# zhenfeizhang/falcon-r1cs

Measured on AMD Instinct MI355X. Metric: falcon1024_verify_with_ntt_r1cs_witnesses_per_sec, higher is better.
Workload: dtype u32

## Files before the change

falcon-r1cs_amd/csrc/frw_fq29.h:

```cpp
#pragma once
#include <hip/hip_runtime.h>
#include <stdint.h>

namespace frw {

constexpr int NLQ = 14;
constexpr uint32_t MQ29 = (1u << 29) - 1u;

struct Fq29 { uint32_t l[NLQ]; };
struct LimbsQ { uint32_t l[NLQ]; };

constexpr uint32_t Q32_[12] = {0xffffaaabu, 0xb9feffffu, 0xb153ffffu, 0x1eabfffeu, 0xf6b0f624u, 0x6730d2a0u,
                               0xf38512bfu, 0x64774b84u, 0x434bacd7u, 0x4b1ba7b6u, 0x397fe69au, 0x1a0111eau};
constexpr LimbsQ make_kq29(uint32_t K)
{
    uint32_t w[14] = {0, 0, 0, 0, 0, 0, 0, 0, 0, 0, 0, 0, 0, 0};
    uint64_t carry = 0;
    for (int k = 0; k < 12; k++) {
        const uint64_t t = (uint64_t)K * Q32_[k] + carry;
        w[k] = (uint32_t)t;
        carry = t >> 32;
    }
    w[12] = (uint32_t)carry;
    LimbsQ r{};
// ... 382 lines not shown
{
    uint32_t y[12], x[12];
    fq_pack(fq_reduce(a), y);
    if (fq_inv_words31(y, x)) return fq_mul(fq_unpack(x), fq_const(FQ29_R3));
    return fq_inv_binary(a);
}
__host__ __device__ inline Fq29 fq_inv_binary(const Fq29 &a)
{
    uint32_t u[12], v[12], x1[12], x2[12];
    fq_pack(fq_reduce(a), u);
#pragma unroll
    for (int k = 0; k < 12; k++) { v[k] = Q32_[k]; x1[k] = k == 0 ? 1u : 0u; x2[k] = 0u; }
#pragma nounroll
    for (int round = 0; round < 2 * 382; round++) {
        uint32_t any = 0;
#pragma unroll
        for (int k = 0; k < 12; k++) any |= u[k];
#if defined(__HIP_DEVICE_COMPILE__)
        if (__builtin_amdgcn_ballot_w64(any != 0) == 0) break;
#else
        if (any == 0) break;
#endif
        const uint32_t odd = 0u - (u[0] & 1u);
        uint32_t d[12], e[12], f[12];
        uint32_t borrow = 0;
#pragma unroll
        for (int k = 0; k < 12; k++) d[k] = sub_b(u[k], v[k], borrow);
        const uint32_t less = 0u - borrow, take = odd & less;
        borrow = 0;
#pragma unroll
        for (int k = 0; k < 12; k++) e[k] = sub_b(x1[k], x2[k], borrow);
        const uint32_t below = 0u - borrow;
        uint32_t carry = 0;
#pragma unroll
        for (int k = 0; k < 12; k++) e[k] = add_c(e[k], Q32_[k] & below, carry);
        borrow = 0;
#pragma unroll
        for (int k = 0; k < 12; k++) f[k] = sub_b(Q32_[k], e[k], borrow);
        borrow = 0;
#pragma unroll
        for (int k = 0; k < 12; k++) {
            const uint32_t neg = sub_b(d[k] ^ less, less, borrow);
            const uint32_t tu = u[k], tx = x1[k];
            u[k] = (odd & neg) | (~odd & tu);
            v[k] = (take & tu) | (~take & v[k]);
            x1[k] = (odd & ((less & f[k]) | (~less & e[k]))) | (~odd & tx);
            x2[k] = (take & tx) | (~take & x2[k]);
        }
        const uint32_t xodd = 0u - (x1[0] & 1u);
        carry = 0;
#pragma unroll
        for (int k = 0; k < 12; k++) x1[k] = add_c(x1[k], Q32_[k] & xodd, carry);
#pragma unroll
        for (int k = 0; k < 12; k++) {
            u[k] = (u[k] >> 1) | (k + 1 < 12 ? u[k + 1] << 31 : 0u);
            x1[k] = (x1[k] >> 1) | (k + 1 < 12 ? x1[k + 1] << 31 : 0u);
        }
    }
    return fq_mul(fq_unpack(x2), fq_const(FQ29_R3));
}

struct Fq2_29 { Fq29 c0, c1; };
__host__ __device__ __forceinline__ Fq2_29 fq2_mul(const Fq2_29 &a, const Fq2_29 &b)
{
    const Fq29 m0 = fq_mul(a.c0, b.c0), m1 = fq_mul(a.c1, b.c1), m2 = fq_mul(fq_add(a.c0, a.c1), fq_add(b.c0, b.c1));
    Fq2_29 r;
    r.c0 = fq_sub<4>(m0, m1);
    r.c1 = fq_sub<4>(fq_sub<4>(m2, m0), m1);
    return r;
}
__host__ __device__ __forceinline__ Fq2_29 fq2_sqr(const Fq2_29 &a)
{
    Fq2_29 r;
    r.c0 = fq_mul(fq_add(a.c0, a.c1), fq_sub<1024>(a.c0, a.c1));
    const Fq29 t = fq_mul(a.c0, a.c1);
    r.c1 = fq_add(t, t);
    return r;
}

struct FqField {
    typedef Fq29 El;
    static constexpr uint32_t K_MUL = 4, K_2MUL = 4, K_X = 16, K_Y = 16;
    static constexpr uint32_t K_AFFINE = K_MUL;
    static constexpr int WORDS = NLQ, ARK_WORDS = 12, LANES = 1;
    __host__ __device__ static __forceinline__ El mul(const El &a, const El &b) { return fq_mul(a, b); }
    __host__ __device__ static __forceinline__ El sqr(const El &a) { return fq_sqr(a); }
    template <uint32_t KC> __host__ __device__ static __forceinline__ El mul_sub(const El &a, const El &b, const El &c, const El &d) { return fq_mul_sub<KC>(a, b, c, d); }
    __host__ __device__ static __forceinline__ El add(const El &a, const El &b) { return fq_add(a, b); }
    template <uint32_t K> __host__ __device__ static __forceinline__ El sub(const El &a, const El &b) { return fq_sub<K>(a, b); }
    template <uint32_t K> __host__ __device__ static __forceinline__ El neg(const El &a) { return fq_neg<K>(a); }
    __host__ __device__ static __forceinline__ El zero() { return fq_zero(); }
    __host__ __device__ static __forceinline__ El one() { return fq_const(FQ29_ONE); }
    __host__ __device__ static __forceinline__ bool is_zero(const El &a) { return fq_is_zero(a); }
    __host__ __device__ static inline El inv(const El &a) { return fq_inv(a); }
    __host__ __device__ static __forceinline__ El from_ark(const uint32_t *w) { return fq_from_ark(w); }
    __host__ __device__ static __forceinline__ void to_ark(const El &a, uint32_t *w) { fq_to_ark(a, w); }
    __host__ __device__ static __forceinline__ void store(const El &a, uint32_t *w)
    {
#pragma unroll
        for (int k = 0; k < NLQ; k++) w[k] = a.l[k];
    }
    __host__ __device__ static __forceinline__ El load(const uint32_t *w)
    {
        El a;
#pragma unroll
        for (int k = 0; k < NLQ; k++) a.l[k] = w[k];
        return a;
    }
};
struct Fq2Field {
    typedef Fq2_29 El;
    static constexpr uint32_t K_MUL = 16, K_2MUL = 64, K_X = 256, K_Y = 64;
    static constexpr uint32_t K_AFFINE = K_MUL;
    static constexpr int WORDS = 2 * NLQ, ARK_WORDS = 24, LANES = 1;
    __host__ __device__ static __forceinline__ El mul(const El &a, const El &b) { return fq2_mul(a, b); }
    __host__ __device__ static __forceinline__ El sqr(const El &a) { return fq2_sqr(a); }
    template <uint32_t KC> __host__ __device__ static __forceinline__ El mul_sub(const El &a, const El &b, const El &c, const El &d)
    {
        return sub<K_MUL>(fq2_mul(a, b), fq2_mul(c, d));
    }
    __host__ __device__ static __forceinline__ El add(const El &a, const El &b) { El r; r.c0 = fq_add(a.c0, b.c0); r.c1 = fq_add(a.c1, b.c1); return r; }
    template <uint32_t K> __host__ __device__ static __forceinline__ El sub(const El &a, const El &b)
    {
        El r; r.c0 = fq_sub<K>(a.c0, b.c0); r.c1 = fq_sub<K>(a.c1, b.c1); return r;
    }
    template <uint32_t K> __host__ __device__ static __forceinline__ El neg(const El &a) { El r; r.c0 = fq_neg<K>(a.c0); r.c1 = fq_neg<K>(a.c1); return r; }
    __host__ __device__ static __forceinline__ El zero() { El r; r.c0 = r.c1 = fq_zero(); return r; }
    __host__ __device__ static __forceinline__ El one() { El r; r.c0 = fq_const(FQ29_ONE); r.c1 = fq_zero(); return r; }
    __host__ __device__ static __forceinline__ bool is_zero(const El &a) { return fq_is_zero(a.c0) && fq_is_zero(a.c1); }
    __host__ __device__ static inline El inv(const El &a)
    {
        const Fq29 n = fq_inv(fq_add(fq_mul(a.c0, a.c0), fq_mul(a.c1, a.c1)));
        El r; r.c0 = fq_mul(a.c0, n); r.c1 = fq_mul(fq_neg<1024>(a.c1), n); return r;
    }
    __host__ __device__ static __forceinline__ El from_ark(const uint32_t *w) { El r; r.c0 = fq_from_ark(w); r.c1 = fq_from_ark(w + 12); return r; }
    __host__ __device__ static __forceinline__ void to_ark(const El &a, uint32_t *w) { fq_to_ark(a.c0, w); fq_to_ark(a.c1, w + 12); }
    __host__ __device__ static __forceinline__ void store(const El &a, uint32_t *w) { FqField::store(a.c0, w); FqField::store(a.c1, w + NLQ); }
    __host__ __device__ static __forceinline__ El load(const uint32_t *w) { El r; r.c0 = FqField::load(w); r.c1 = FqField::load(w + NLQ); return r; }
};

#if defined(__HIPCC__)
struct Fq2Half { Fq29 v; };
__device__ __forceinline__ uint32_t pair_swap_u32(uint32_t x)
{
    return (uint32_t)__builtin_amdgcn_mov_dpp((int)x, 0xB1 , 0xf, 0xf, true);
}
__device__ __forceinline__ Fq29 pair_swap(const Fq29 &a)
{
    Fq29 r;
#pragma unroll
    for (int i = 0; i < NLQ; i++) r.l[i] = pair_swap_u32(a.l[i]);
    return r;
}
__device__ __forceinline__ Fq29 fq_select(bool take_a, const Fq29 &a, const Fq29 &b)
{
    Fq29 r;
#pragma unroll
    for (int i = 0; i < NLQ; i++) r.l[i] = take_a ? a.l[i] : b.l[i];
    return r;
}
struct Fq2PairField {
    typedef Fq2Half El;
    static constexpr uint32_t K_MUL = 4, K_2MUL = 16, K_X = 256, K_Y = 64;
    static constexpr uint32_t K_AFFINE = 16;
    static constexpr int WORDS = 2 * NLQ, ARK_WORDS = 24, LANES = 2;
    __device__ static __forceinline__ bool odd() { return (threadIdx.x & 1u) != 0; }
    __device__ static __forceinline__ El mul(const El &a, const El &b)
    {
        const Fq29 ap = pair_swap(a.v), bp = pair_swap(b.v);
        const bool o = odd();
        const Fq29 x = fq_select(o, ap, a.v), y = fq_select(o, a.v, fq_neg<1024>(ap));
        uint64_t col[2 * NLQ];
        fq_mul2_cols(x, b.v, y, bp, col);
        El r;
        r.v = fq_reduce_cols(col);
        return r;
    }
    __device__ static __forceinline__ El sqr(const El &a)
    {
        const Fq29 ap = pair_swap(a.v);
        const bool o = odd();
        const Fq29 x = fq_add(a.v, fq_select(o, a.v, ap)), y = fq_select(o, ap, fq_sub<1024>(a.v, ap));
        El r;
        r.v = fq_mul(x, y);
        return r;
    }
    template <uint32_t KC> __device__ static __forceinline__ El mul_sub(const El &a, const El &b, const El &c, const El &d)
    {
        return sub<K_MUL>(mul(a, b), mul(c, d));
    }
    __device__ static __forceinline__ El add(const El &a, const El &b) { El r; r.v = fq_add(a.v, b.v); return r; }
    template <uint32_t K> __device__ static __forceinline__ El sub(const El &a, const El &b) { El r; r.v = fq_sub<K>(a.v, b.v); return r; }
    template <uint32_t K> __device__ static __forceinline__ El neg(const El &a) { El r; r.v = fq_neg<K>(a.v); return r; }
    __device__ static __forceinline__ El zero() { El r; r.v = fq_zero(); return r; }
    __device__ static __forceinline__ El one() { El r; r.v = fq_select(odd(), fq_zero(), fq_const(FQ29_ONE)); return r; }
    __device__ static __forceinline__ bool is_zero(const El &a)
    {
        const uint32_t mine = fq_is_zero(a.v) ? 1u : 0u;
        return (mine & pair_swap_u32(mine)) != 0;
    }
    __device__ static inline El inv(const El &a)
    {
        const Fq29 sq = fq_sqr(a.v);
        const Fq29 n = fq_inv(fq_add(sq, pair_swap(sq)));
        El r;
        r.v = fq_mul(fq_select(odd(), fq_neg<1024>(a.v), a.v), n);
        return r;
    }
    __device__ static __forceinline__ El from_ark(const uint32_t *w) { El r; r.v = fq_from_ark(w + (odd() ? 12 : 0)); return r; }
    __device__ static __forceinline__ void to_ark(const El &a, uint32_t *w) { fq_to_ark(a.v, w + (odd() ? 12 : 0)); }
    __device__ static __forceinline__ void store(const El &a, uint32_t *w) { FqField::store(a.v, w + (odd() ? NLQ : 0)); }
    __device__ static __forceinline__ El load(const uint32_t *w) { El r; r.v = FqField::load(w + (odd() ? NLQ : 0)); return r; }
};
#endif

constexpr LimbsQ G1_GEN_X29 = {{0x0af58fd1u, 0x1662a68eu, 0x07d2c530u, 0x08993c24u, 0x1e4f4756u, 0x0c5f7ae2u, 0x0f589991u,
                                0x00dc570eu, 0x121b54f5u, 0x05242b28u, 0x17442464u, 0x0ee8a0cdu, 0x1f591099u, 0x00000009u}};
constexpr LimbsQ G1_GEN_Y29 = {{0x1cd65f60u, 0x1919ce91u, 0x0da44145u, 0x0810b2ccu, 0x08f38c44u, 0x00629241u, 0x0f521d8cu,
                                0x0529cbadu, 0x0506077fu, 0x191b2712u, 0x0c587ccbu, 0x1017da2fu, 0x1c72eafau, 0x0000000bu}};
constexpr LimbsQ G2_GEN_X0_29 = {{0x085d7b9eu, 0x0d352838u, 0x124c5276u, 0x1748cfe0u, 0x10081802u, 0x0bfc6540u, 0x01ac1784u,
                                   0x11aab37fu, 0x08f338c1u, 0x19443e06u, 0x1cc29975u, 0x0a0da681u, 0x0a53e408u, 0x00000004u}};
constexpr LimbsQ G2_GEN_X1_29 = {{0x0ba695cbu, 0x1034485fu, 0x124f6eb5u, 0x0778336bu, 0x1e170b2du, 0x12164b09u, 0x1d34eb65u,
                                   0x10a72ef2u, 0x07b96a4eu, 0x194de314u, 0x0fd4fa4au, 0x0178f021u, 0x10455591u, 0x0000000bu}};
constexpr LimbsQ G2_GEN_Y0_29 = {{0x1ec793b8u, 0x1780929bu, 0x0cdd65c4u, 0x126ca64fu, 0x0f9f2f6bu, 0x09485ce0u, 0x0621fd94u,
                                   0x1e0e7efdu, 0x09ba1f86u, 0x06d0a458u, 0x1f790335u, 0x0af83757u, 0x00c11d05u, 0x0000000cu}};
constexpr LimbsQ G2_GEN_Y1_29 = {{0x014e8093u, 0x07f6c9aau, 0x19bd3883u, 0x156ca3e1u, 0x0e34898fu, 0x0840b6feu, 0x0594f57du,
                                   0x149969ecu, 0x12886b3eu, 0x1cbcbe34u, 0x1cae2f62u, 0x08f5e851u, 0x187a6c6cu, 0x00000003u}};

constexpr LimbsQ G1_ENDO_BETA29 = {{0x1195dfebu, 0x1b04e484u, 0x06026044u, 0x086070a2u, 0x1fd68858u, 0x137e9670u, 0x06871e67u,
                                    0x1e736664u, 0x083b24f6u, 0x08a70373u, 0x02a012fdu, 0x0112f94bu, 0x18a2733cu, 0x00000003u}};

template <class F> struct AffineT { typename F::El x, y; bool inf; };
template <class F> struct XyzzT { typename F::El x, y, zz, zzz; bool inf; };

template <class F> __host__ __device__ __forceinline__ XyzzT<F> pt_identity()
{
    XyzzT<F> r;
    r.x = r.y = r.zz = r.zzz = F::zero();
    r.inf = true;
    return r;
}
template <class F> __host__ __device__ __forceinline__ XyzzT<F> pt_from_affine(const AffineT<F> &p)
{
    XyzzT<F> r;
    r.x = p.x; r.y = p.y; r.zz = r.zzz = F::one();
    r.inf = p.inf;
    return r;
}
template <class F> __host__ __device__ inline XyzzT<F> pt_double(const XyzzT<F> &p)
{
    if (p.inf) return p;
    const auto u = F::add(p.y, p.y);
    const auto v = F::sqr(u), w = F::mul(u, v);
    const auto s = F::mul(p.x, v);
    const auto xx = F::sqr(p.x);
    const auto m = F::add(F::add(xx, xx), xx);
    XyzzT<F> r;
    r.x = F::template sub<F::K_2MUL>(F::sqr(m), F::add(s, s));
    r.y = F::template mul_sub<F::K_MUL>(m, F::template sub<F::K_X>(s, r.x), w, p.y);
    r.zz = F::mul(v, p.zz);
    r.zzz = F::mul(w, p.zzz);
    r.inf = false;
    return r;
}
template <class F> __host__ __device__ __forceinline__ XyzzT<F> pt_add_affine(const XyzzT<F> &p, const AffineT<F> &q)
{
    if (q.inf) return p;
    if (p.inf) return pt_from_affine(q);
    const auto u2 = F::mul(q.x, p.zz), s2 = F::mul(q.y, p.zzz);
    const auto pp_ = F::template sub<F::K_X>(u2, p.x);
    const auto rr = F::template sub<F::K_Y>(s2, p.y);
    if (F::is_zero(pp_)) {
        if (F::is_zero(rr)) return pt_double(pt_from_affine(q));
        return pt_identity<F>();
    }
    const auto pp = F::sqr(pp_), ppp = F::mul(pp_, pp), qq = F::mul(p.x, pp);
    XyzzT<F> r;
    r.x = F::template sub<F::K_2MUL>(F::template sub<F::K_MUL>(F::sqr(rr), ppp), F::add(qq, qq));
    r.y = F::template mul_sub<F::K_Y>(rr, F::template sub<F::K_X>(qq, r.x), p.y, ppp);
    r.zz = F::mul(p.zz, pp);
    r.zzz = F::mul(p.zzz, ppp);
    r.inf = false;
    return r;
}
template <class F> __host__ __device__ inline XyzzT<F> pt_add(const XyzzT<F> &p, const XyzzT<F> &q)
{
    if (q.inf) return p;
    if (p.inf) return q;
    const auto u1 = F::mul(p.x, q.zz), u2 = F::mul(q.x, p.zz), s1 = F::mul(p.y, q.zzz), s2 = F::mul(q.y, p.zzz);
    const auto pp_ = F::template sub<F::K_MUL>(u2, u1), rr = F::template sub<F::K_MUL>(s2, s1);
    if (F::is_zero(pp_)) {
        if (F::is_zero(rr)) return pt_double(p);
        return pt_identity<F>();
    }
    const auto pp = F::sqr(pp_), ppp = F::mul(pp_, pp), qq = F::mul(u1, pp);
    XyzzT<F> r;
    r.x = F::template sub<F::K_2MUL>(F::template sub<F::K_MUL>(F::sqr(rr), ppp), F::add(qq, qq));
    r.y = F::template mul_sub<F::K_MUL>(rr, F::template sub<F::K_X>(qq, r.x), s1, ppp);
    r.zz = F::mul(F::mul(p.zz, q.zz), pp);
    r.zzz = F::mul(F::mul(p.zzz, q.zzz), ppp);
    r.inf = false;
    return r;
}
template <class F> __host__ __device__ inline AffineT<F> pt_to_affine(const XyzzT<F> &p)
{
    AffineT<F> r;
    r.inf = p.inf;
    if (p.inf) { r.x = r.y = F::zero(); return r; }
    const auto inv = F::inv(F::mul(p.zz, p.zzz));
    r.x = F::mul(p.x, F::mul(inv, p.zzz));
    r.y = F::mul(p.y, F::mul(inv, p.zz));
    return r;
}

typedef AffineT<FqField> G1Affine29;
typedef XyzzT<FqField> G1Xyzz;
typedef AffineT<Fq2Field> G2Affine29;
typedef XyzzT<Fq2Field> G2Xyzz;
__host__ __device__ __forceinline__ G1Xyzz g1_identity() { return pt_identity<FqField>(); }
__host__ __device__ __forceinline__ G1Xyzz g1_from_affine(const G1Affine29 &p) { return pt_from_affine(p); }
__host__ __device__ inline G1Xyzz g1_double(const G1Xyzz &p) { return pt_double(p); }
__host__ __device__ inline G1Xyzz g1_add_affine(const G1Xyzz &p, const G1Affine29 &q) { return pt_add_affine(p, q); }
__host__ __device__ inline G1Xyzz g1_add(const G1Xyzz &p, const G1Xyzz &q) { return pt_add(p, q); }
__host__ __device__ inline G1Affine29 g1_to_affine(const G1Xyzz &p) { return pt_to_affine(p); }

}
```

falcon-r1cs_amd/csrc/frw_msm.hip:

```cpp
#include <hip/hip_runtime.h>
#include <stdint.h>
#include <algorithm>
#include <cstdlib>
#include <cstring>
#include <functional>
#include <new>
#include <mutex>
#include <vector>
#include "../../include/frw.h"
#include "frw_device.h"
#include "frw_fq29.h"
#include "frw_quad.h"
#include "frw_fr29.h"

namespace frw {

constexpr int MSM_C = 16;
constexpr int MSM_W = 16;
constexpr int MSM_BUCKETS = 1 << (MSM_C - 1);
constexpr int MSM_FOLD1_THREADS = 4096;
constexpr int MSM_FOLD_THREADS = 512;
template <class F> struct Grp {
    static constexpr int PT_WORDS = 2 * F::WORDS, BK_WORDS = 4 * F::WORDS + 4, ARK_WORDS = 2 * F::ARK_WORDS;
    static constexpr uint32_t K_AFFINE_Y = F::K_AFFINE;
// ... 358 lines not shown
#pragma unroll
        for (int k = 0; k < WIDE_TILE / 1024; k++) {
            const uint32_t i = tile0 + t + 1024u * k;
            dv[k] = i < hi ? digits[j * n + i] : 0;
            if (dv[k]) atomicAdd(&tcount[((uint32_t)(dv[k] < 0 ? -dv[k] : dv[k]) - 1u) >> 10], 1u);
        }
        __syncthreads();
        {
            uint32_t incl = t < WIDE_BINS ? tcount[t] : 0u;
            const uint32_t own = incl, lane = t & 63;
#pragma unroll
            for (int off = 1; off < 64; off <<= 1) {
                const uint32_t v = __shfl_up(incl, off, 64);
                if (lane >= (uint32_t)off) incl += v;
            }
            if (t < WIDE_BINS && lane == 63) wtotal[t >> 6] = incl;
            __syncthreads();
            if (t < WIDE_BINS) {
                uint32_t before = 0;
                for (uint32_t w_ = 0; w_ < (t >> 6); w_++) before += wtotal[w_];
                tstart[t] = before + incl - own;
            }
            __syncthreads();
        }
#pragma unroll
        for (int k = 0; k < WIDE_TILE / 1024; k++) {
            if (!dv[k]) continue;
            const uint32_t i = tile0 + t + 1024u * k, m = (uint32_t)(dv[k] < 0 ? -dv[k] : dv[k]) - 1u, bin = m >> 10;
            const uint32_t pos = tstart[bin] + atomicAdd(&tfill[bin], 1u);
            stage[pos] = make_uint2(i | (dv[k] < 0 ? 0x80000000u : 0u), m & (WIDE_BIN_BUCKETS - 1));
            sbin[pos] = (uint16_t)bin;
        }
        __syncthreads();
        const uint32_t total = tstart[WIDE_BINS - 1] + tcount[WIDE_BINS - 1];
        for (uint32_t p = t; p < total; p += 1024) {
            const uint32_t bin = sbin[p];
            coarse[gpos[bin] + (p - tstart[bin])] = stage[p];
        }
        __syncthreads();
        if (t < WIDE_BINS) gpos[t] += tcount[t];
        __syncthreads();
    }
}
constexpr int WIDE_PARTS = 32;
static_assert(WIDE_ALL_BINS % 8 == 0, "bins go to the XCDs eight at a time");
struct WidePart { size_t g; uint32_t part, lo, hi; };
__device__ __forceinline__ WidePart wide_part_of(uint32_t w, const uint32_t *__restrict__ bin_count)
{
    WidePart p;
    const uint32_t q = w >> 3;
    p.part = q % WIDE_PARTS;
    p.g = (size_t)(q / WIDE_PARTS) * 8 + (w & 7);
    const uint32_t cnt = bin_count[p.g];
    p.lo = (uint32_t)((uint64_t)cnt * p.part / WIDE_PARTS);
    p.hi = (uint32_t)((uint64_t)cnt * (p.part + 1) / WIDE_PARTS);
    return p;
}
__global__ __launch_bounds__(1024) void msm_wide_bucket_hist_kernel(const uint2 *__restrict__ coarse, const uint32_t *__restrict__ bin_count,
                                                                    const unsigned long long *__restrict__ bin_start, uint32_t *__restrict__ part_hist)
{
    __shared__ uint32_t hist[WIDE_BIN_BUCKETS];
    const WidePart p = wide_part_of(blockIdx.x, bin_count);
    const uint2 *src = coarse + bin_start[p.g];
    hist[threadIdx.x] = 0;
    __syncthreads();
    for (uint32_t i = p.lo + threadIdx.x; i < p.hi; i += 1024) atomicAdd(&hist[src[i].y], 1u);
    __syncthreads();
    part_hist[(p.g * WIDE_PARTS + p.part) * WIDE_BIN_BUCKETS + threadIdx.x] = hist[threadIdx.x];
}
__global__ __launch_bounds__(1024) void msm_wide_bucket_parts_kernel(uint32_t *__restrict__ part_hist, uint32_t *__restrict__ counts)
{
    const size_t g = blockIdx.x;
    uint32_t run = 0;
    for (int part = 0; part < WIDE_PARTS; part++) {
        uint32_t *h = part_hist + (g * WIDE_PARTS + part) * WIDE_BIN_BUCKETS + threadIdx.x;
        const uint32_t c = *h;
        *h = run;
        run += c;
    }
    counts[g * WIDE_BIN_BUCKETS + threadIdx.x] = run;
}
__global__ __launch_bounds__(1024) void msm_wide_bucket_scatter_kernel(const uint2 *__restrict__ coarse, const uint32_t *__restrict__ bin_count,
                                                                       const unsigned long long *__restrict__ bin_start, const uint32_t *__restrict__ offsets,
                                                                       const uint32_t *__restrict__ part_hist, const unsigned long long *__restrict__ row_start,
                                                                       uint32_t *__restrict__ entries)
{
    __shared__ uint32_t cursor[WIDE_BIN_BUCKETS];
    const WidePart p = wide_part_of(blockIdx.x, bin_count);
    const uint2 *src = coarse + bin_start[p.g];
    cursor[threadIdx.x] = offsets[p.g * WIDE_BIN_BUCKETS + threadIdx.x] + part_hist[(p.g * WIDE_PARTS + p.part) * WIDE_BIN_BUCKETS + threadIdx.x];
    __syncthreads();
    uint32_t *ent = entries + row_start[p.g >> 5];
    constexpr int U = 8;
    for (uint32_t i0 = p.lo + threadIdx.x; i0 < p.hi; i0 += 1024 * U) {
        uint2 e[U];
#pragma unroll
        for (int k = 0; k < U; k++) e[k] = i0 + 1024u * k < p.hi ? src[i0 + 1024u * k] : make_uint2(0u, 0u);
#pragma unroll
        for (int k = 0; k < U; k++)
            if (i0 + 1024u * k < p.hi) ent[atomicAdd(&cursor[e[k].y], 1u)] = e[k].x;
    }
}
template <class F>
__global__ __launch_bounds__(64) void msm_wide_window_kernel(const uint32_t *__restrict__ s1 , const uint32_t *__restrict__ s0,
                                                             uint32_t *__restrict__ window_sums )
{
    __builtin_amdgcn_s_setprio(2);
    constexpr int BW = Grp<F>::BK_WORDS;
    if (threadIdx.x >= (unsigned)F::LANES) return;
    const size_t j = blockIdx.x;
    XyzzT<F> run = pt_identity<F>(), weighted = pt_identity<F>(), plain = load_bucket<F>(s1 + (j * WIDE_H) * BW);
    for (int hi = WIDE_H - 1; hi >= 1; hi--) {
        run = pt_add(run, load_bucket<F>(s0 + (j * WIDE_H + hi) * BW));
        weighted = pt_add(weighted, run);
        plain = pt_add(plain, load_bucket<F>(s1 + (j * WIDE_H + hi) * BW));
    }
    for (int k = 0; k < MSM_C - 1; k++) weighted = pt_double(weighted);
    store_bucket<F>(window_sums + j * BW, pt_add(plain, weighted));
}

__global__ __launch_bounds__(256) void msm_slice_offsets_kernel(uint32_t *__restrict__ slice_hist, uint32_t *__restrict__ counts, int slices)
{
    const size_t sig = blockIdx.y;
    const uint32_t b = blockIdx.x * 256 + threadIdx.x;
    uint32_t *h = slice_hist + sig * slices * (size_t)MSM_BUCKETS + b;
    uint32_t run = 0;
#pragma unroll 4
    for (int s_ = 0; s_ < slices; s_++) {
        const uint32_t c = h[(size_t)s_ * MSM_BUCKETS];
        h[(size_t)s_ * MSM_BUCKETS] = run;
        run += c;
    }
    counts[sig * MSM_BUCKETS + b] = run;
}

__global__ __launch_bounds__(1024) void msm_scan_kernel(const uint32_t *__restrict__ counts, uint32_t *__restrict__ offsets)
{
    __shared__ uint32_t part[1024];
    const size_t sig = blockIdx.x;
    const uint32_t *cnt = counts + sig * MSM_BUCKETS;
    const int t = threadIdx.x;
    constexpr int PER = MSM_BUCKETS / 1024;
    uint32_t local[PER], s = 0;
#pragma unroll
    for (int k = 0; k < PER; k++) { local[k] = s; s += cnt[t * PER + k]; }
    part[t] = s;
    __syncthreads();
    for (int off = 1; off < 1024; off <<= 1) {
        const uint32_t v = t >= off ? part[t - off] : 0u;
        __syncthreads();
        part[t] += v;
        __syncthreads();
    }
    const uint32_t base = part[t] - s;
#pragma unroll
    for (int k = 0; k < PER; k++) offsets[sig * MSM_BUCKETS + t * PER + k] = base + local[k];
}

__global__ __launch_bounds__(1024) void msm_scatter_kernel(uint32_t n, const uint32_t *__restrict__ scalars, size_t sig_stride_words,
                                                           int montgomery, const uint32_t *__restrict__ offsets,
                                                           const uint32_t *__restrict__ slice_hist, uint32_t *__restrict__ entries, int bare)
{
    __shared__ uint32_t cursor[MSM_BUCKETS];
    const size_t row = blockIdx.y, sig = bare ? 0 : row;
    const uint32_t slices = gridDim.x, slice = blockIdx.x, per = (n + slices - 1) / slices;
    const uint32_t lo = slice * per, hi = lo + per < n ? lo + per : n;
    const uint32_t *first = slice_hist + (row * slices + slice) * MSM_BUCKETS, *off = offsets + row * MSM_BUCKETS;
    for (int b = threadIdx.x; b < MSM_BUCKETS; b += 1024) cursor[b] = off[b] + first[b];
    __syncthreads();
    uint32_t *ent = entries + row * (bare ? (size_t)n : (size_t)MSM_W * n);
    for (uint32_t i = lo + threadIdx.x; i < hi; i += 1024) {
        int d[MSM_W];
        if (scalar_digits(scalars + sig * sig_stride_words + (size_t)i * 8, montgomery, d, !bare)) continue;
        if (bare) {
            const int v = msm_digit_of(d, (uint32_t)row);
            if (v) ent[atomicAdd(&cursor[(uint32_t)(v < 0 ? -v : v) - 1u], 1u)] = i | (v < 0 ? 0x80000000u : 0u);
            continue;
        }
#pragma unroll
        for (int j = 0; j < MSM_W; j++) {
            if (!d[j]) continue;
            const uint32_t b = (uint32_t)(d[j] < 0 ? -d[j] : d[j]) - 1u;
            ent[atomicAdd(&cursor[b], 1u)] = ((uint32_t)j * n + i) | (d[j] < 0 ? 0x80000000u : 0u);
        }
    }
}

constexpr int MSM_SIZE_CLASSES = 1024;
constexpr int MSM_MAX_ITEMS = 131072;
constexpr int MSM_MAX_ITEMS_LARGE = 32768 + (32768 * 24 * 2 / 3) / 32 * 33 + 64;
static_assert(MSM_MAX_ITEMS_LARGE % 64 == 0 && MSM_MAX_ITEMS >= 32768 + (32768 * 4 * 2 / 3) / 32 * 33 + 64, "whole wavefronts; the finest split fits");
__host__ __device__ constexpr uint32_t msm_max_items(uint32_t n, bool bare = false)
{
    return !bare && n > (1u << 18) ? (uint32_t)MSM_MAX_ITEMS_LARGE : (uint32_t)MSM_MAX_ITEMS;
}
__device__ __forceinline__ uint32_t msm_split_of(uint32_t total, uint32_t finer)
{
    const uint32_t s = (uint32_t)(((uint64_t)total * 3 + 2 * MSM_BUCKETS - 1) / (2 * MSM_BUCKETS)) / finer;
    return s < 32u ? 32u : s;
}
__global__ __launch_bounds__(1024) void msm_order_kernel(const uint32_t *__restrict__ counts, const uint32_t *__restrict__ offsets,
                                                         uint32_t *__restrict__ order, uint32_t *__restrict__ item_first ,
                                                         uint32_t *__restrict__ items ,
                                                         uint32_t *__restrict__ item_count , uint32_t finer, uint32_t max_items)
{
    __shared__ uint32_t hist[MSM_SIZE_CLASSES];
    const size_t sig = blockIdx.x;
    const uint32_t *cnt = counts + sig * MSM_BUCKETS;
    uint32_t *ord = order + sig * MSM_BUCKETS;
    const int t = threadIdx.x;
    hist[t] = 0;
    __syncthreads();
    auto cls = [](uint32_t c) { return c >= (uint32_t)MSM_SIZE_CLASSES ? 0u : (uint32_t)(MSM_SIZE_CLASSES - 1) - c; };
    for (int b = t; b < MSM_BUCKETS; b += 1024) atomicAdd(&hist[cls(cnt[b])], 1u);
    __syncthreads();
    const uint32_t mine = hist[t];
    __syncthreads();
    for (int off = 1; off < 1024; off <<= 1) {
        const uint32_t v = t >= off ? hist[t - off] : 0u;
        __syncthreads();
        hist[t] += v;
        __syncthreads();
    }
    const uint32_t excl = hist[t] - mine;
    __syncthreads();
    hist[t] = excl;
    __syncthreads();
    for (int b = t; b < MSM_BUCKETS; b += 1024) ord[atomicAdd(&hist[cls(cnt[b])], 1u)] = (uint32_t)b;
    __threadfence_block();
    __syncthreads();
    const uint32_t total = offsets[sig * MSM_BUCKETS + MSM_BUCKETS - 1] + cnt[MSM_BUCKETS - 1], split = msm_split_of(total, finer);
    constexpr int PER = MSM_BUCKETS / 1024;
    uint32_t k[PER], local = 0;
#pragma unroll
    for (int j = 0; j < PER; j++) {
        const uint32_t c = cnt[ord[t * PER + j]];
        k[j] = c <= split ? 1u : (c + split - 1) / split;
        local += k[j];
    }
    hist[t] = local;
    __syncthreads();
    for (int off = 1; off < 1024; off <<= 1) {
        const uint32_t v = t >= off ? hist[t - off] : 0u;
        __syncthreads();
        hist[t] += v;
        __syncthreads();
    }
    uint32_t pos = hist[t] - local;
    if (t == 1023) item_count[sig] = hist[t] < max_items ? hist[t] : max_items;
#pragma unroll
    for (int j = 0; j < PER; j++) {
        const uint32_t b = ord[t * PER + j];
        item_first[sig * MSM_BUCKETS + b] = pos;
        for (uint32_t c = 0; c < k[j] && pos + c < max_items; c++) {
            uint32_t *it = items + (sig * (size_t)max_items + pos + c) * 2;
            it[0] = b;
            it[1] = c;
        }
        pos += k[j];
    }
}

template <class F, bool PREFETCH>
__global__ __launch_bounds__(64, 2) void msm_bucket_kernel(MsmDev m, const uint32_t *__restrict__ offsets, const uint32_t *__restrict__ counts,
                                                           const uint32_t *__restrict__ items, const uint32_t *__restrict__ item_count,
                                                           const uint32_t *__restrict__ entries, uint32_t *__restrict__ partial_items, uint32_t finer,
                                                           uint32_t max_items, size_t ent_stride ,
                                                           const unsigned long long *__restrict__ row_base )
{
    constexpr int PW = Grp<F>::PT_WORDS;
    const size_t sig = blockIdx.y;
    const uint32_t it = blockIdx.x * 64 + threadIdx.x;
    if (it >= item_count[sig]) return;
    const uint2 item = *(const uint2 *)(items + (sig * (size_t)max_items + it) * 2);
    const uint32_t b = item.x, chunk = item.y;
    const uint32_t c = counts[sig * MSM_BUCKETS + b];
    const uint32_t total = offsets[sig * MSM_BUCKETS + MSM_BUCKETS - 1] + counts[sig * MSM_BUCKETS + MSM_BUCKETS - 1], split = msm_split_of(total, finer);
    const uint32_t k = c <= split ? 1u : (c + split - 1) / split;
    const uint32_t lo = (uint32_t)((uint64_t)c * chunk / k), cnt = (uint32_t)((uint64_t)c * (chunk + 1) / k) - lo;
    const uint32_t *ent = entries + (row_base ? (size_t)row_base[sig] : sig * ent_stride) + offsets[sig * MSM_BUCKETS + b] + lo;
    XyzzT<F> acc = pt_identity<F>();
    if (PREFETCH) {
        uint32_t e = cnt ? ent[0] : 0u;
        AffineT<F> p = load_row<F>(m.table + (size_t)(e & 0x7fffffffu) * PW);
        for (uint32_t j = 0; j < cnt; j++) {
            const uint32_t e_next = j + 1 < cnt ? ent[j + 1] : e;
            const AffineT<F> p_next = load_row<F>(m.table + (size_t)(e_next & 0x7fffffffu) * PW);
            if (e >> 31) p.y = F::template neg<Grp<F>::K_AFFINE_Y>(p.y);
            acc = pt_add_affine(acc, p);
            e = e_next;
            p = p_next;
        }
    } else {
        for (uint32_t j = 0; j < cnt; j++) {
            const uint32_t e = ent[j];
            AffineT<F> p = load_row<F>(m.table + (size_t)(e & 0x7fffffffu) * PW);
            if (e >> 31) p.y = F::template neg<Grp<F>::K_AFFINE_Y>(p.y);
            acc = pt_add_affine(acc, p);
        }
    }
    store_bucket<F>(partial_items + (sig * (size_t)max_items + it) * (size_t)Grp<F>::BK_WORDS, acc);
}

template <class F>
__global__ __launch_bounds__(64) void msm_horner_kernel(const uint32_t *__restrict__ sums, int windows, int window_bits,
                                                        uint32_t *__restrict__ out , int xyzz_out,
                                                        uint32_t out_step = 1 )
{
    __builtin_amdgcn_s_setprio(2);
    constexpr int BW = Grp<F>::BK_WORDS;
    if (threadIdx.x >= (unsigned)F::LANES) return;
    const uint32_t *src = sums + (size_t)blockIdx.x * windows * BW;
    XyzzT<F> acc = load_bucket<F>(src + (size_t)(windows - 1) * BW);
    for (int j = windows - 2; j >= 0; j--) {
        for (int k = 0; k < window_bits; k++) acc = pt_double(acc);
        acc = pt_add(acc, load_bucket<F>(src + (size_t)j * BW));
    }
    if (xyzz_out) store_bucket<F>(out + (size_t)blockIdx.x * out_step * BW, acc);
    else store_ark_point<F>(out + (size_t)blockIdx.x * Grp<F>::ARK_WORDS, pt_to_affine(acc));
}
template <int PT_WORDS_>
__global__ __launch_bounds__(1024) void live_rows_kernel(const uint32_t *__restrict__ rows, uint32_t n, uint32_t *__restrict__ block_counts ,
                                                         uint32_t *__restrict__ index )
{
    __shared__ uint32_t wave_total[16];
    const uint32_t i = blockIdx.x * 1024 + threadIdx.x, lane = threadIdx.x & 63, wave = threadIdx.x >> 6;
    uint32_t any = 0;
    if (i < n) {
        const uint4 *v = (const uint4 *)(rows + (size_t)i * PT_WORDS_);
#pragma unroll
        for (int k = 0; k < PT_WORDS_ / 4; k++) { const uint4 w = v[k]; any |= w.x | w.y | w.z | w.w; }
    }
    const unsigned long long ballot = __builtin_amdgcn_ballot_w64(any != 0);
    if (lane == 0) wave_total[wave] = (uint32_t)__popcll(ballot);
    __syncthreads();
    uint32_t before = 0, total = 0;
    for (uint32_t w = 0; w < 16; w++) { before += w < wave ? wave_total[w] : 0u; total += wave_total[w]; }
    if (!index) {
        if (threadIdx.x == 0) block_counts[blockIdx.x] = total;
        return;
    }
    if (any) index[block_counts[blockIdx.x] + before + (uint32_t)__popcll(ballot & ((1ull << lane) - 1))] = i;
}
__global__ __launch_bounds__(1024) void live_rows_scan_kernel(uint32_t *__restrict__ block_counts, uint32_t blocks, uint32_t *__restrict__ total)
{
    __shared__ uint32_t run_total[1024];
    const uint32_t per = (blocks + 1023) / 1024, lo = threadIdx.x * per, hi = lo + per < blocks ? lo + per : blocks;
    uint32_t sum = 0;
    for (uint32_t b = lo; b < hi; b++) sum += block_counts[b];
    run_total[threadIdx.x] = sum;
    __syncthreads();
    uint32_t before = 0;
    for (uint32_t t = 0; t < threadIdx.x; t++) before += run_total[t];
    for (uint32_t b = lo; b < hi; b++) { const uint32_t c = block_counts[b]; block_counts[b] = before; before += c; }
    if (threadIdx.x == 1023) *total = before;
}

template <class F>
__global__ __launch_bounds__(64, 2) void msm_combine_kernel(const uint32_t *__restrict__ offsets, const uint32_t *__restrict__ counts,
                                                            const uint32_t *__restrict__ item_first, const uint32_t *__restrict__ partial_items,
                                                            uint32_t *__restrict__ buckets, uint32_t finer, uint32_t max_items)
{
    __builtin_amdgcn_s_setprio(2);
    constexpr int BW = Grp<F>::BK_WORDS;
    const size_t sig = blockIdx.y;
    const uint32_t b = blockIdx.x * 64 + threadIdx.x;
    const uint32_t c = counts[sig * MSM_BUCKETS + b];
    const uint32_t total = offsets[sig * MSM_BUCKETS + MSM_BUCKETS - 1] + counts[sig * MSM_BUCKETS + MSM_BUCKETS - 1], split = msm_split_of(total, finer);
    const uint32_t k = c <= split ? 1u : (c + split - 1) / split;
    const uint32_t *src = partial_items + (sig * (size_t)max_items + item_first[sig * MSM_BUCKETS + b]) * (size_t)BW;
    XyzzT<F> acc = load_bucket<F>(src);
    for (uint32_t j = 1; j < k; j++) acc = pt_add(acc, load_bucket<F>(src + (size_t)j * BW));
    store_bucket<F>(buckets + (sig * MSM_BUCKETS + b) * (size_t)BW, acc);
}

template <class F>
__global__ __launch_bounds__(64, 2) void msm_ones_kernel(MsmDev m, const uint32_t *__restrict__ ones_count, const uint32_t *__restrict__ ones_list,
                                                         uint32_t *__restrict__ partial )
{
    const size_t sig = blockIdx.y;
    const uint32_t nthreads = gridDim.x * 64;
    const uint32_t t = blockIdx.x * 64 + threadIdx.x, cnt = ones_count[sig];
    const uint32_t *list = ones_list + sig * m.n;
    XyzzT<F> acc = pt_identity<F>();
    for (uint32_t k = t; k < cnt; k += nthreads)
        acc = pt_add_affine(acc, load_row<F>(m.table + (size_t)list[k] * Grp<F>::PT_WORDS));
    store_bucket<F>(partial + (sig * MSM_FOLD1_THREADS + t) * (size_t)Grp<F>::BK_WORDS, acc);
}

template <class F, int LOG_CHUNK>
__global__ __launch_bounds__(64, 2) void msm_fold1_kernel(const uint32_t *__restrict__ buckets, uint32_t *__restrict__ partial,
                                                          uint32_t *__restrict__ partial_plain )
{
    __builtin_amdgcn_s_setprio(2);
    constexpr int BW = Grp<F>::BK_WORDS, CHUNK = 1 << LOG_CHUNK;
    const size_t sig = blockIdx.y;
    const int g = blockIdx.x * 64 + threadIdx.x;
    const uint32_t *bk = buckets + (sig * MSM_BUCKETS + (size_t)g * CHUNK) * BW;
    XyzzT<F> run = pt_identity<F>(), sum = pt_identity<F>();
    for (int k = CHUNK - 1; k >= 0; k--) {
        run = pt_add(run, load_bucket<F>(bk + (size_t)k * BW));
        sum = pt_add(sum, run);
    }
    XyzzT<F> mult = pt_identity<F>();
    for (int bit = 14 - LOG_CHUNK; bit >= 0; bit--) {
        mult = pt_double(mult);
        if ((g >> bit) & 1) mult = pt_add(mult, run);
    }
    for (int k = 0; k < LOG_CHUNK; k++) mult = pt_double(mult);
    sum = pt_add(sum, mult);
    uint32_t *mine = partial + (sig * MSM_FOLD1_THREADS + g) * (size_t)BW;
    sum = pt_add(sum, load_bucket<F>(mine));
    store_bucket<F>(mine, sum);
    if (partial_plain) store_bucket<F>(partial_plain + (sig * MSM_FOLD1_THREADS + g) * (size_t)BW, run);
}
template <class F>
__global__ __launch_bounds__(MSM_FOLD_THREADS) void msm_fold2_kernel(const uint32_t *__restrict__ partial, int each,
                                                                     uint32_t *__restrict__ out , int xyzz_out)
{
    __builtin_amdgcn_s_setprio(2);
    constexpr int SLOT = 4 * F::WORDS + 1, BW = Grp<F>::BK_WORDS;
    __shared__ uint32_t lds[MSM_FOLD_THREADS / 2 * SLOT];
    const size_t sig = blockIdx.x;
    const int t = threadIdx.x;
    const uint32_t *src = partial + (sig * MSM_FOLD1_THREADS + (size_t)t * each) * BW;
    XyzzT<F> sum = load_bucket<F>(src);
    for (int k = 1; k < each; k++) sum = pt_add(sum, load_bucket<F>(src + (size_t)k * BW));
    for (int stride = MSM_FOLD_THREADS / 2; stride >= 1; stride >>= 1) {
        if (t >= stride && t < 2 * stride) store_bucket<F>(lds + (t - stride) * SLOT, sum);
        __syncthreads();
        if (t < stride) sum = pt_add(sum, load_bucket<F>(lds + t * SLOT));
        __syncthreads();
    }
    if (t == 0) {
        if (xyzz_out) store_bucket<F>(out + sig * BW, sum);
        else store_ark_point<F>(out + sig * Grp<F>::ARK_WORDS, pt_to_affine(sum));
    }
}

constexpr int NMSM_C = 8, NMSM_W = 32, NMSM_BUCKETS = 128;
__host__ __device__ constexpr uint32_t nmsm_slices(uint32_t n) { return n > (1u << 18) ? 128u : 16u; }
__device__ __forceinline__ void wave_append(bool want, uint32_t *__restrict__ count, uint32_t *__restrict__ list, uint32_t value)
{
    const unsigned long long mask = __builtin_amdgcn_ballot_w64(want);
    if (!mask) return;
    const uint32_t lane = __builtin_amdgcn_mbcnt_hi((uint32_t)(mask >> 32), __builtin_amdgcn_mbcnt_lo((uint32_t)mask, 0u));
    const int leader = __builtin_ctzll(mask);
    uint32_t base = 0;
    if ((int)(threadIdx.x & 63) == leader) base = atomicAdd(count, (uint32_t)__popcll(mask));
    base = __shfl(base, leader, 64);
    if (want) list[base + lane] = value;
}
constexpr int NMSM_TARGET_ITEMS_MIN = 2048, NMSM_TARGET_ITEMS_MAX = 65536;
__host__ __device__ constexpr uint32_t nmsm_target_items(uint32_t n)
{
    const uint32_t t = (n / 128 + 2047) / 2048 * 2048;
    return t < (uint32_t)NMSM_TARGET_ITEMS_MIN ? (uint32_t)NMSM_TARGET_ITEMS_MIN : t > (uint32_t)NMSM_TARGET_ITEMS_MAX ? (uint32_t)NMSM_TARGET_ITEMS_MAX : t;
}
__host__ __device__ constexpr uint32_t nmsm_max_items(uint32_t n) { return nmsm_target_items(n) + 256; }
constexpr int NMSM_ONES_MAX = 4096, NMSM_ONES_MAX_LARGE = 65536;
__host__ __device__ constexpr uint32_t nmsm_ones_max(uint32_t n) { return n > (1u << 18) ? (uint32_t)NMSM_ONES_MAX_LARGE : (uint32_t)NMSM_ONES_MAX; }
__device__ __forceinline__ bool scalar_digits8(const uint32_t *src, int montgomery, int (&d)[NMSM_W])
{
    const Fr8 w = scalar_canonical(src, montgomery);
    if (w.l[0] == 1u && !(w.l[1] | w.l[2] | w.l[3] | w.l[4] | w.l[5] | w.l[6] | w.l[7])) return true;
    int carry = 0;
#pragma unroll
    for (int j = 0; j < NMSM_W; j++) {
        int v = (int)((w.l[j >> 2] >> (8 * (j & 3))) & 0xffu) + carry;
        carry = 0;
        if (j + 1 < NMSM_W && v > NMSM_BUCKETS) { v -= 1 << NMSM_C; carry = 1; }
        d[j] = v;
    }
    return false;
}
__device__ __forceinline__ uint32_t nmsm_split_of(uint32_t total, uint32_t target)
{
    const uint32_t s = (total + target - 1) / target;
    return s < 32u ? 32u : s;
}
__global__ __launch_bounds__(1024) void nmsm_hist_kernel(uint32_t n, const uint32_t *__restrict__ scalars, size_t sig_stride_words, int montgomery,
                                                         uint32_t *__restrict__ slice_hist ,
                                                         uint32_t *__restrict__ ones_count , uint32_t *__restrict__ ones_list ,
                                                         int ones_as_mask)
{
    __shared__ uint32_t hist[NMSM_BUCKETS];
    const size_t sig = blockIdx.y;
    const uint32_t slices = gridDim.x, slice = blockIdx.x, per = (n + slices - 1) / slices;
    const uint32_t lo = slice * per, hi = lo + per < n ? lo + per : n;
    if (threadIdx.x < NMSM_BUCKETS) hist[threadIdx.x] = 0;
    __syncthreads();
    for (uint32_t i = lo + threadIdx.x; i < hi; i += 1024) {
        int d[NMSM_W];
        if (scalar_digits8(scalars + sig * sig_stride_words + (size_t)i * 8, montgomery, d)) {
            if (ones_as_mask) atomicOr(&ones_list[sig * n + (i >> 5)], 1u << (i & 31));
            else ones_list[sig * n + atomicAdd(&ones_count[sig], 1u)] = i;
            continue;
        }
#pragma unroll
        for (int j = 0; j < NMSM_W; j++)
            if (d[j]) atomicAdd(&hist[(d[j] < 0 ? -d[j] : d[j]) - 1], 1u);
    }
    __syncthreads();
    if (threadIdx.x < NMSM_BUCKETS) slice_hist[(sig * slices + slice) * NMSM_BUCKETS + threadIdx.x] = hist[threadIdx.x];
}
__global__ __launch_bounds__(NMSM_BUCKETS) void nmsm_plan_kernel(uint32_t *__restrict__ slice_hist, uint32_t *__restrict__ counts, uint32_t *__restrict__ offsets,
                                                                 uint32_t *__restrict__ item_first, uint32_t *__restrict__ items ,
                                                                 uint32_t *__restrict__ item_count , uint32_t target, uint32_t max_items, uint32_t slices)
{
    __shared__ uint32_t scan[NMSM_BUCKETS];
    const size_t sig = blockIdx.x;
    const int b = threadIdx.x;
    uint32_t *h = slice_hist + sig * slices * (size_t)NMSM_BUCKETS + b;
    uint32_t c = 0;
    for (uint32_t s_ = 0; s_ < slices; s_++) {
        const uint32_t v = h[(size_t)s_ * NMSM_BUCKETS];
        h[(size_t)s_ * NMSM_BUCKETS] = c;
        c += v;
    }
    auto inclusive_scan = [&](uint32_t mine) {
        scan[b] = mine;
        __syncthreads();
        for (int off = 1; off < NMSM_BUCKETS; off <<= 1) {
            const uint32_t v = b >= off ? scan[b - off] : 0u;
            __syncthreads();
            scan[b] += v;
            __syncthreads();
        }
        const uint32_t r = scan[b];
        __syncthreads();
        return r;
    };
    const uint32_t incl = inclusive_scan(c);
    scan[b] = incl;
    __syncthreads();
    const uint32_t total = scan[NMSM_BUCKETS - 1], split = nmsm_split_of(total, target);
    __syncthreads();
    counts[sig * NMSM_BUCKETS + b] = c;
    offsets[sig * NMSM_BUCKETS + b] = incl - c;
    const uint32_t k = c <= split ? 1u : (c + split - 1) / split;
    const uint32_t kincl = inclusive_scan(k), first = kincl - k;
    item_first[sig * NMSM_BUCKETS + b] = first;
    if (b == NMSM_BUCKETS - 1) item_count[sig] = kincl;
    for (uint32_t part = 0; part < k; part++) items[sig * (size_t)max_items + first + part] = (uint32_t)b | (part << 8);
}
__global__ __launch_bounds__(1024) void nmsm_scatter_kernel(uint32_t n, const uint32_t *__restrict__ scalars, size_t sig_stride_words, int montgomery,
                                                            const uint32_t *__restrict__ offsets, const uint32_t *__restrict__ slice_hist,
                                                            uint32_t *__restrict__ entries )
{
    __shared__ uint32_t cursor[NMSM_BUCKETS];
    const size_t sig = blockIdx.y;
    const uint32_t slices = gridDim.x, slice = blockIdx.x, per = (n + slices - 1) / slices;
    const uint32_t lo = slice * per, hi = lo + per < n ? lo + per : n;
    if (threadIdx.x < NMSM_BUCKETS)
        cursor[threadIdx.x] = offsets[sig * NMSM_BUCKETS + threadIdx.x] + slice_hist[(sig * slices + slice) * NMSM_BUCKETS + threadIdx.x];
    __syncthreads();
    uint32_t *ent = entries + sig * (size_t)NMSM_W * n;
    for (uint32_t i = lo + threadIdx.x; i < hi; i += 1024) {
        int d[NMSM_W];
        if (scalar_digits8(scalars + sig * sig_stride_words + (size_t)i * 8, montgomery, d)) continue;
#pragma unroll
        for (int j = 0; j < NMSM_W; j++) {
            if (!d[j]) continue;
            const uint32_t b = (uint32_t)(d[j] < 0 ? -d[j] : d[j]) - 1u;
            ent[atomicAdd(&cursor[b], 1u)] = ((uint32_t)j * n + i) | (d[j] < 0 ? 0x80000000u : 0u);
        }
    }
}
__global__ __launch_bounds__(1024) void nmsm_hist_bare_kernel(uint32_t n, const uint32_t *__restrict__ scalars, int montgomery,
                                                              uint32_t *__restrict__ slice_hist ,
                                                              uint32_t *__restrict__ ones_count , uint32_t *__restrict__ ones_list ,
                                                              const uint32_t *__restrict__ index)
{
    constexpr uint32_t ONES_CAP = 4096;
    __shared__ uint32_t hist[NMSM_W * NMSM_BUCKETS];
    __shared__ uint32_t ones_buf[ONES_CAP];
    __shared__ uint32_t ones_fill, ones_base;
    const uint32_t slices = gridDim.x, slice = blockIdx.x, per = (n + slices - 1) / slices;
    const uint32_t lo = slice * per, hi = lo + per < n ? lo + per : n;
    for (int b = threadIdx.x; b < NMSM_W * NMSM_BUCKETS; b += 1024) hist[b] = 0;
    if (threadIdx.x == 0) ones_fill = 0;
    __syncthreads();
    auto flush = [&](uint32_t fill) {
        if (threadIdx.x == 0 && fill) ones_base = atomicAdd(&ones_count[0], fill);
        __syncthreads();
        for (uint32_t t = threadIdx.x; t < fill; t += 1024) ones_list[ones_base + t] = ones_buf[t];
        __syncthreads();
        if (threadIdx.x == 0) ones_fill = 0;
        __syncthreads();
    };
    for (uint32_t k0 = lo; k0 < hi; k0 += 1024) {
        const uint32_t k = k0 + threadIdx.x;
        bool one = false;
        if (k < hi) {
            const uint32_t i = index ? index[k] : k;
            int d[NMSM_W];
            one = scalar_digits8(scalars + (size_t)i * 8, montgomery, d);
            if (one) {
                ones_buf[atomicAdd(&ones_fill, 1u)] = i;
            } else {
#pragma unroll
                for (int j = 0; j < NMSM_W; j++)
                    if (d[j]) atomicAdd(&hist[j * NMSM_BUCKETS + (d[j] < 0 ? -d[j] : d[j]) - 1], 1u);
            }
        }
        __syncthreads();
        const uint32_t fill = ones_fill;
        __syncthreads();
        if (fill > ONES_CAP - 1024) flush(fill);
    }
    flush(ones_fill);
    __syncthreads();
    for (int b = threadIdx.x; b < NMSM_W * NMSM_BUCKETS; b += 1024)
        slice_hist[((size_t)(b / NMSM_BUCKETS) * slices + slice) * NMSM_BUCKETS + (b % NMSM_BUCKETS)] = hist[b];
}
__global__ __launch_bounds__(64) void nmsm_entry_base_kernel(const uint32_t *__restrict__ counts, const uint32_t *__restrict__ offsets,
                                                             unsigned long long *__restrict__ entry_base )
{
    if (threadIdx.x) return;
    unsigned long long run = 0;
    for (int w = 0; w < NMSM_W; w++) {
        entry_base[w] = run;
        run += (unsigned long long)offsets[w * NMSM_BUCKETS + NMSM_BUCKETS - 1] + counts[w * NMSM_BUCKETS + NMSM_BUCKETS - 1];
    }
}
__global__ __launch_bounds__(1024) void nmsm_scatter_bare_kernel(uint32_t n, const uint32_t *__restrict__ scalars, int montgomery,
                                                                 const uint32_t *__restrict__ offsets ,
                                                                 const uint32_t *__restrict__ slice_hist,
                                                                 const unsigned long long *__restrict__ entry_base, uint32_t *__restrict__ entries,
                                                                 const uint32_t *__restrict__ index)
{
    __shared__ uint32_t cursor[NMSM_W * NMSM_BUCKETS];
    __shared__ unsigned long long base[NMSM_W];
    const uint32_t slices = gridDim.x, slice = blockIdx.x, per = (n + slices - 1) / slices;
    const uint32_t lo = slice * per, hi = lo + per < n ? lo + per : n;
    for (int b = threadIdx.x; b < NMSM_W * NMSM_BUCKETS; b += 1024)
        cursor[b] = offsets[b] + slice_hist[((size_t)(b / NMSM_BUCKETS) * slices + slice) * NMSM_BUCKETS + (b % NMSM_BUCKETS)];
    if (threadIdx.x < NMSM_W) base[threadIdx.x] = entry_base[threadIdx.x];
    __syncthreads();
    for (uint32_t k = lo + threadIdx.x; k < hi; k += 1024) {
        const uint32_t i = index ? index[k] : k;
        int d[NMSM_W];
        if (scalar_digits8(scalars + (size_t)i * 8, montgomery, d)) continue;
#pragma unroll
        for (int j = 0; j < NMSM_W; j++) {
            if (!d[j]) continue;
            const uint32_t b = (uint32_t)(d[j] < 0 ? -d[j] : d[j]) - 1u;
            entries[base[j] + atomicAdd(&cursor[j * NMSM_BUCKETS + b], 1u)] = i | (d[j] < 0 ? 0x80000000u : 0u);
        }
    }
}
template <class F, bool PREFETCH>
__global__ __launch_bounds__(64, F::LANES > 1 ? 1 : 2) void nmsm_bucket_kernel(NmsmTables tables, const uint32_t *__restrict__ offsets, const uint32_t *__restrict__ counts,
                                                            const uint32_t *__restrict__ items, const uint32_t *__restrict__ item_count,
                                                            const uint32_t *__restrict__ entries, uint32_t *__restrict__ partial_items,
                                                            uint32_t target, uint32_t max_items,
                                                            const unsigned long long *__restrict__ entry_base )
{
    __builtin_amdgcn_s_setprio(2);
    constexpr int PW = Grp<F>::PT_WORDS;
    const size_t slot = blockIdx.y;
    size_t sig;
    const MsmDev m = tables.of(blockIdx.y, sig);
    const uint32_t it = (blockIdx.x * 64 + threadIdx.x) / F::LANES;
    if (it >= item_count[sig]) return;
    const uint32_t item = items[sig * (size_t)max_items + it], b = item & (NMSM_BUCKETS - 1), part = item >> 8;
    const uint32_t c = counts[sig * NMSM_BUCKETS + b];
    const uint32_t total = offsets[sig * NMSM_BUCKETS + NMSM_BUCKETS - 1] + counts[sig * NMSM_BUCKETS + NMSM_BUCKETS - 1], split = nmsm_split_of(total, target);
    const uint32_t k = c <= split ? 1u : (c + split - 1) / split;
    const uint32_t lo = (uint32_t)((uint64_t)c * part / k), cnt = (uint32_t)((uint64_t)c * (part + 1) / k) - lo;
    const uint32_t *ent = entries + (entry_base ? (size_t)entry_base[sig] : sig * (size_t)NMSM_W * m.n) + offsets[sig * NMSM_BUCKETS + b] + lo;
    XyzzT<F> acc = pt_identity<F>();
    if (PREFETCH) {
        uint32_t e = cnt ? ent[0] : 0u;
        AffineT<F> p = load_row<F>(m.table + (size_t)(e & 0x7fffffffu) * PW);
        for (uint32_t j = 0; j < cnt; j++) {
            const uint32_t e_next = j + 1 < cnt ? ent[j + 1] : e;
            const AffineT<F> p_next = load_row<F>(m.table + (size_t)(e_next & 0x7fffffffu) * PW);
            if (e >> 31) p.y = F::template neg<Grp<F>::K_AFFINE_Y>(p.y);
            acc = pt_add_affine(acc, p);
            e = e_next;
            p = p_next;
        }
    } else {
        for (uint32_t j = 0; j < cnt; j++) {
            const uint32_t e = ent[j];
            AffineT<F> p = load_row<F>(m.table + (size_t)(e & 0x7fffffffu) * PW);
            if (e >> 31) p.y = F::template neg<Grp<F>::K_AFFINE_Y>(p.y);
            acc = pt_add_affine(acc, p);
        }
    }
    store_bucket<F>(partial_items + (slot * (size_t)max_items + it) * (size_t)Grp<F>::BK_WORDS, acc);
}
template <class F>
__global__ __launch_bounds__(64, F::LANES > 1 ? 1 : 2) void nmsm_ones_kernel(NmsmTables tables, const uint32_t *__restrict__ ones_count, const uint32_t *__restrict__ ones_list,
                                                          uint32_t *__restrict__ partial_ones , uint32_t groups_stride,
                                                          uint32_t row_step )
{
    __builtin_amdgcn_s_setprio(2);
    constexpr int SLOT = 4 * F::WORDS + 1, PER = 64 / F::LANES;
    __shared__ uint32_t lds[32 * SLOT];
    const size_t slot = blockIdx.y;
    size_t sig;
    const MsmDev m = tables.of(blockIdx.y * row_step, sig);
    const uint32_t nthreads = gridDim.x * PER, t = blockIdx.x * PER + threadIdx.x / F::LANES;
    const uint32_t *list = ones_list + sig * m.n;
    XyzzT<F> acc = pt_identity<F>();
    if (m.ones_table) {
        const uint32_t groups = (m.n + 7) / 8;
        for (uint32_t g = t; g < groups; g += nthreads) {
            const uint32_t byte = (list[g >> 2] >> (8 * (g & 3))) & 0xffu;
            if (byte) acc = pt_add_affine(acc, load_row<F>(m.ones_table + ((size_t)g * 255 + (byte - 1)) * Grp<F>::PT_WORDS));
        }
    } else {
        const uint32_t cnt = ones_count[sig];
        for (uint32_t k = t; k < cnt; k += nthreads)
            acc = pt_add_affine(acc, load_row<F>(m.table + (size_t)list[k] * Grp<F>::PT_WORDS));
    }
    const int lane = threadIdx.x / F::LANES;
    for (int stride = PER / 2; stride >= 1; stride >>= 1) {
        if (lane >= stride && lane < 2 * stride) store_bucket<F>(lds + (lane - stride) * SLOT, acc);
        __syncthreads();
        if (lane < stride) acc = pt_add(acc, load_bucket<F>(lds + lane * SLOT));
        __syncthreads();
    }
    if (lane == 0) store_bucket<F>(partial_ones + (slot * (size_t)groups_stride + blockIdx.x) * (size_t)Grp<F>::BK_WORDS, acc);
}
template <class F> struct BulkPolicy { typedef F type; };
template <> struct BulkPolicy<Fq2Field> { typedef Fq2PairField type; };
template <class F>
__global__ __launch_bounds__(64, F::LANES > 1 ? 1 : 2) void nmsm_ones_fold_kernel(const uint32_t *__restrict__ partial_ones, uint32_t groups, uint32_t groups_stride,
                                                               uint32_t *__restrict__ folded )
{
    __builtin_amdgcn_s_setprio(2);
    constexpr int SLOT = 4 * F::WORDS + 1, BW = Grp<F>::BK_WORDS, PER = 64 / F::LANES;
    __shared__ uint32_t lds[32 * SLOT];
    const size_t sig = blockIdx.y;
    const uint32_t g = blockIdx.x, lane = threadIdx.x / F::LANES;
    const uint32_t *src = partial_ones + sig * (size_t)groups_stride * BW;
    XyzzT<F> acc = pt_identity<F>();
    for (uint32_t k = g + 64 * lane; k < groups; k += 64 * PER) acc = pt_add(acc, load_bucket<F>(src + (size_t)k * BW));
    for (int stride = PER / 2; stride >= 1; stride >>= 1) {
        if ((int)lane >= stride && (int)lane < 2 * stride) store_bucket<F>(lds + (lane - stride) * SLOT, acc);
        __syncthreads();
        if ((int)lane < stride) acc = pt_add(acc, load_bucket<F>(lds + lane * SLOT));
        __syncthreads();
    }
    if (lane == 0) store_bucket<F>(folded + (sig * 64 + g) * (size_t)BW, acc);
}
template <class F>
__global__ __launch_bounds__(64, F::LANES > 1 ? 1 : 2) void nmsm_combine_kernel(const uint32_t *__restrict__ counts, const uint32_t *__restrict__ offsets,
                                                             const uint32_t *__restrict__ item_first, const uint32_t *__restrict__ partial_items,
                                                             uint32_t *__restrict__ buckets , uint32_t target, uint32_t max_items,
                                                             uint32_t sigs)
{
    __builtin_amdgcn_s_setprio(2);
    constexpr int SLOT = 4 * F::WORDS + 1, BW = Grp<F>::BK_WORDS, PER = 64 / F::LANES;
    __shared__ uint32_t lds[32 * SLOT];
    const size_t slot = blockIdx.y, sig = slot % sigs;
    const uint32_t b = blockIdx.x, lane = threadIdx.x / F::LANES;
    const uint32_t c = counts[sig * NMSM_BUCKETS + b];
    const uint32_t total = offsets[sig * NMSM_BUCKETS + NMSM_BUCKETS - 1] + counts[sig * NMSM_BUCKETS + NMSM_BUCKETS - 1], split = nmsm_split_of(total, target);
    const uint32_t k = c <= split ? 1u : (c + split - 1) / split;
    const uint32_t *src = partial_items + (slot * (size_t)max_items + item_first[sig * NMSM_BUCKETS + b]) * (size_t)BW;
    XyzzT<F> acc = pt_identity<F>();
    for (uint32_t j = lane; j < k; j += PER) acc = pt_add(acc, load_bucket<F>(src + (size_t)j * BW));
    for (int stride = PER / 2; stride >= 1; stride >>= 1) {
        if ((int)lane >= stride && (int)lane < 2 * stride) store_bucket<F>(lds + (lane - stride) * SLOT, acc);
        __syncthreads();
        if ((int)lane < stride) acc = pt_add(acc, load_bucket<F>(lds + lane * SLOT));
        __syncthreads();
    }
    if (lane == 0) store_bucket<F>(buckets + (slot * NMSM_BUCKETS + b) * (size_t)BW, acc);
}

template <class F>
__global__ __launch_bounds__(64) void nmsm_finish_kernel(const uint32_t *__restrict__ counts, const uint32_t *__restrict__ offsets,
                                                         const uint32_t *__restrict__ item_first, const uint32_t *__restrict__ partial_items,
                                                         const uint32_t *__restrict__ buckets ,
                                                         const uint32_t *__restrict__ partial_ones ,
                                                         int ones_groups, uint32_t ones_stride, uint32_t target, uint32_t max_items,
                                                         uint32_t *__restrict__ out , int xyzz_out,
                                                         uint32_t sigs, int ones_window0 )
{
    __builtin_amdgcn_s_setprio(2);
    constexpr int SLOT = 4 * F::WORDS + 1, BW = Grp<F>::BK_WORDS, PER = 64 / F::LANES, NB = NMSM_BUCKETS / PER;
    constexpr int LOG_PER = PER == 64 ? 6 : 5, LOG_NB = NB == 2 ? 1 : 2;
    static_assert(PER * NB == NMSM_BUCKETS && (1 << LOG_PER) == PER && (1 << LOG_NB) == NB, "64 or 32 chains of 2 or 4 buckets");
    __shared__ uint32_t lds[NMSM_BUCKETS * SLOT];
    __shared__ uint32_t longest[NB];
    const size_t slot = blockIdx.x, sig = slot % sigs;
    const int i = threadIdx.x / F::LANES;
    const uint32_t *src[NB];
    uint32_t mine[NB];
    if (threadIdx.x < NB) longest[threadIdx.x] = 1;
    __syncthreads();
#pragma unroll
    for (int k = 0; k < NB; k++) {
        const int b = i * NB + k;
        if (buckets) {
            src[k] = buckets + (slot * NMSM_BUCKETS + b) * (size_t)BW;
            mine[k] = 1;
        } else {
            const uint32_t c = counts[sig * NMSM_BUCKETS + b];
            const uint32_t total = offsets[sig * NMSM_BUCKETS + NMSM_BUCKETS - 1] + counts[sig * NMSM_BUCKETS + NMSM_BUCKETS - 1], split = nmsm_split_of(total, target);
            mine[k] = c <= split ? 1u : (c + split - 1) / split;
            src[k] = partial_items + (slot * (size_t)max_items + item_first[sig * NMSM_BUCKETS + b]) * (size_t)BW;
            atomicMax(&longest[k], mine[k]);
        }
    }
    __syncthreads();
    uint32_t phase0 = 0;
#pragma unroll
    for (int k = 0; k < NB; k++) phase0 += longest[k] + 1;
    const int ones_steps = (ones_groups + PER - 1) / PER;
    const uint32_t at_local = phase0, at_reload = at_local + (NB - 1) + 1, at_scan = at_reload + 1, at_weight = at_scan + LOG_PER,
                   at_final = at_weight + LOG_NB, at_ones = at_final + 1, at_tree = at_ones + ones_steps, steps = at_tree + LOG_PER;
    XyzzT<F> sum = pt_identity<F>();
    for (uint32_t step = 0; step < steps; step++) {
        int store_slot = -1;
        bool reset = false, add = false;
        const uint32_t *p = lds;
        if (step < phase0) {
            uint32_t s = step;
            int k = NB - 1;
#pragma unroll
            for (int kk = NB - 1; kk >= 1; kk--)
                if (k == kk && s >= longest[kk] + 1) { s -= longest[kk] + 1; k = kk - 1; }
            const uint32_t *sp = src[0];
            uint32_t mk = mine[0], lk = longest[0];
#pragma unroll
            for (int kk = 1; kk < NB; kk++)
                if (k == kk) { sp = src[kk]; mk = mine[kk]; lk = longest[kk]; }
            if (s < lk) { add = s < mk; p = sp + (size_t)s * BW; }
            else store_slot = i * NB + k;
        } else if (step < at_reload - 1) {
            add = true; p = lds + (i * NB + 1 + (int)(step - at_local)) * SLOT;
        } else if (step == at_reload - 1) {
            store_slot = i * NB + 1;
        } else if (step == at_reload) {
            reset = true; add = true; p = lds + (i * NB) * SLOT;
        } else if (step < at_weight) {
            const int off = 1 << (step - at_scan);
            store_slot = i * NB;
            add = i + off < PER; p = lds + ((i + off) * NB) * SLOT;
        } else if (step < at_final) {
            store_slot = i * NB;
            add = true; p = lds + (i * NB) * SLOT;
        } else if (step == at_final) {
            reset = i == 0;
            add = true; p = lds + (i * NB + 1) * SLOT;
        } else if (step < at_tree) {
            const int g = i + PER * (int)(step - at_ones);
            const size_t ones_row = ones_window0 ? slot / sigs : slot;
            add = g < ones_groups && !(ones_window0 && sig != 0); p = partial_ones + (ones_row * (size_t)ones_stride + (size_t)g) * BW;
        } else {
            const int stride = PER >> (step - at_tree + 1);
            if (i >= stride && i < 2 * stride) store_slot = (i - stride) * NB;
            add = i < stride; p = lds + (i * NB) * SLOT;
        }
        if (store_slot >= 0) store_bucket<F>(lds + store_slot * SLOT, sum);
        __syncthreads();
        if (reset) sum = pt_identity<F>();
        if (add) sum = pt_add(sum, load_bucket<F>(p));
        __syncthreads();
    }
    if (i == 0) {
        if (xyzz_out) store_bucket<F>(out + slot * BW, sum);
        else store_ark_point<F>(out + slot * Grp<F>::ARK_WORDS, pt_to_affine(sum));
    }
}

constexpr int FB_WINDOWS = 32, FB_DIGITS = 256;
template <class F> __device__ __forceinline__ AffineT<F> group_generator();
template <> __device__ __forceinline__ AffineT<FqField> group_generator<FqField>()
{
    AffineT<FqField> g;
    g.x = fq_const(G1_GEN_X29); g.y = fq_const(G1_GEN_Y29); g.inf = false;
    return g;
}
template <> __device__ __forceinline__ AffineT<Fq2Field> group_generator<Fq2Field>()
{
    AffineT<Fq2Field> g;
    g.x.c0 = fq_const(G2_GEN_X0_29); g.x.c1 = fq_const(G2_GEN_X1_29); g.y.c0 = fq_const(G2_GEN_Y0_29); g.y.c1 = fq_const(G2_GEN_Y1_29);
    g.inf = false;
    return g;
}
template <class F>
__global__ __launch_bounds__(64) void fixed_base_table_kernel(uint32_t *__restrict__ table )
{
    const int id = blockIdx.x * 64 + threadIdx.x, w = id >> 8, d = id & 255;
    if (w >= FB_WINDOWS) return;
    const AffineT<F> g = group_generator<F>();
    XyzzT<F> acc = pt_identity<F>();
    for (int bit = 7; bit >= 0; bit--) {
        acc = pt_double(acc);
        if ((d >> bit) & 1) acc = pt_add_affine(acc, g);
    }
    for (int k = 0; k < 8 * w; k++) acc = pt_double(acc);
    store_row<F>(table + (size_t)id * Grp<F>::PT_WORDS, pt_to_affine(acc));
}
template <class F>
__global__ __launch_bounds__(64) void fixed_base_kernel(size_t count, const uint32_t *__restrict__ scalars ,
                                                        const uint32_t *__restrict__ table, uint32_t *__restrict__ out )
{
    const size_t i = (size_t)blockIdx.x * 64 + threadIdx.x;
    if (i >= count) return;
    const Fr8 k = fr_load(scalars + i * 8);
    XyzzT<F> acc = pt_identity<F>();
    for (int w = 0; w < FB_WINDOWS; w++) {
        const uint32_t d = (k.l[w >> 2] >> (8 * (w & 3))) & 255u;
        if (d) acc = pt_add_affine(acc, load_row<F>(table + ((size_t)w * FB_DIGITS + d) * Grp<F>::PT_WORDS));
    }
    store_ark_point<F>(out + i * Grp<F>::ARK_WORDS, pt_to_affine(acc));
}
constexpr int FBW_WINDOWS = 16, FBW_DIGITS = 65536;
template <class F>
__global__ __launch_bounds__(64) void fixed_base_window_gens_kernel(uint32_t *__restrict__ gens )
{
    if (threadIdx.x || blockIdx.x) return;
    XyzzT<F> acc = pt_from_affine(group_generator<F>());
    for (int w = 0; w < FBW_WINDOWS; w++) {
        store_row<F>(gens + (size_t)w * Grp<F>::PT_WORDS, pt_to_affine(acc));
        for (int k = 0; k < 16; k++) acc = pt_double(acc);
    }
}
template <class F>
__global__ __launch_bounds__(64) void fixed_base_wide_table_kernel(const uint32_t *__restrict__ gens, uint32_t *__restrict__ table )
{
    const uint32_t id = blockIdx.x * 64 + threadIdx.x, w = id >> 16, d = id & 65535u;
    if (w >= (uint32_t)FBW_WINDOWS) return;
    const AffineT<F> g = load_row<F>(gens + (size_t)w * Grp<F>::PT_WORDS);
    XyzzT<F> acc = pt_identity<F>();
    for (int bit = 15; bit >= 0; bit--) {
        acc = pt_double(acc);
        if ((d >> bit) & 1u) acc = pt_add_affine(acc, g);
    }
    store_row<F>(table + (size_t)id * Grp<F>::PT_WORDS, pt_to_affine(acc));
}
template <class F, bool ARK_OUT>
__global__ __launch_bounds__(64) void fixed_base_wide_kernel(size_t count, const uint32_t *__restrict__ scalars ,
                                                             const uint32_t *__restrict__ table, uint32_t *__restrict__ out)
{
    const size_t i = ((size_t)blockIdx.x * 64 + threadIdx.x) / F::LANES;
    if (i >= count) return;
    const Fr8 k = fr_load(scalars + i * 8);
    XyzzT<F> acc = pt_identity<F>();
    for (int w = 0; w < FBW_WINDOWS; w++) {
        const uint32_t d = (k.l[w >> 1] >> (16 * (w & 1))) & 65535u;
        if (d) acc = pt_add_affine(acc, load_row<F>(table + ((size_t)w * FBW_DIGITS + d) * Grp<F>::PT_WORDS));
    }
    if (ARK_OUT) store_ark_point<F>(out + i * Grp<F>::ARK_WORDS, pt_to_affine(acc));
    else store_row<F>(out + i * Grp<F>::PT_WORDS, pt_to_affine(acc));
}

}

#if !defined(FRW_MSM_PROBE)
struct frw_msm {
    int device;
    int group;
    int window_bits;
    bool bare = false;
    bool wide = false;
    uint64_t row_lo = 0;
    frw::MsmDev dev;
    void *table;
    void *ones_table;
};

namespace {
using frw::FqField;
using frw::Fq2Field;
template <class F> struct MsmBufs {
    uint32_t *counts, *offsets, *order, *item_first, *item_count, *ones_count, *items, *buckets, *partial, *partial_items, *entries, *ones_list, *end;
    int16_t *digits;
    uint32_t max_items;
    size_t ent_stride, ones_stride;
};
template <class F> MsmBufs<F> msm_carve(void *ws, size_t rows, uint32_t n, bool bare)
{
    constexpr size_t BW = frw::Grp<F>::BK_WORDS;
    static_assert((size_t)frw::MSM_SLICES * 4 <= BW * 4, "the slice histograms borrow the buckets' memory");
    static_assert((size_t)frw::MSM_SLICES_LONE * frw::MSM_BUCKETS <= (size_t)frw::MSM_MAX_ITEMS * BW, "... or, for a lone signature, the work items'");
    MsmBufs<F> b;
    b.max_items = frw::msm_max_items(n, bare);
    b.ent_stride = bare ? (size_t)n : (size_t)frw::MSM_W * n;
    b.ones_stride = bare ? 0 : (size_t)n;
    b.counts = (uint32_t *)ws;
    b.offsets = b.counts + rows * frw::MSM_BUCKETS;
    b.order = b.offsets + rows * frw::MSM_BUCKETS;
    b.item_first = b.order + rows * frw::MSM_BUCKETS;
    b.item_count = b.item_first + rows * frw::MSM_BUCKETS;
    b.ones_count = b.item_count + rows * 4;
    b.items = b.ones_count + rows * 4;
    b.buckets = b.items + rows * (size_t)b.max_items * 2;
    b.partial = b.buckets + rows * (size_t)frw::MSM_BUCKETS * BW;
    b.partial_items = b.partial + rows * (size_t)frw::MSM_FOLD1_THREADS * BW;
    b.entries = b.partial_items + rows * (size_t)b.max_items * BW;
    b.ones_list = b.entries + rows * b.ent_stride;
    b.end = b.ones_list + rows * b.ones_stride;
    b.digits = nullptr;
    if (bare) {
        b.digits = (int16_t *)b.end;
        b.end += ((size_t)frw::MSM_W * n * 2 + 3) / 4;
    }
    return b;
}
constexpr uint32_t MSM_WIDE_FROM_DEFAULT = (1u << 26) - 1;
static uint32_t msm_wide_from()
{
    static const uint32_t v = [] {
        const char *e = getenv("FRW_BARE_WIDE_FROM_LOG2");
        const int lg = e ? atoi(e) : 0;
        return lg >= 10 && lg <= 31 ? ((uint32_t)1 << lg) - 1 : MSM_WIDE_FROM_DEFAULT;
    }();
    return v;
}
template <class F> struct MsmWideBufs {
    MsmBufs<F> rows;
    uint32_t *partial_plain, *slice_hist, *bin_count, *row_count, *s1, *s0, *window_sums, *entries, *end;
    unsigned long long *row_start, *bin_start;
    uint2 *coarse;
    int32_t *digits;
};
template <class F> MsmWideBufs<F> msm_carve_wide(void *ws, uint32_t n)
{
    constexpr size_t BW = frw::Grp<F>::BK_WORDS, R = frw::WIDE_ROWS;
    MsmWideBufs<F> w;
    MsmBufs<F> &b = w.rows;
    b.max_items = frw::WIDE_MAX_ITEMS;
    b.ent_stride = 0; b.ones_stride = 0; b.digits = nullptr;
    b.counts = (uint32_t *)ws;
    b.offsets = b.counts + R * frw::MSM_BUCKETS;
    b.order = b.offsets + R * frw::MSM_BUCKETS;
    b.item_first = b.order + R * frw::MSM_BUCKETS;
    b.item_count = b.item_first + R * frw::MSM_BUCKETS;
    b.ones_count = b.item_count + R * 4;
    b.items = b.ones_count + R * 4;
    b.buckets = b.items + R * (size_t)b.max_items * 2;
    b.partial = b.buckets + R * (size_t)frw::MSM_BUCKETS * BW;
    w.partial_plain = b.partial + R * (size_t)frw::MSM_FOLD1_THREADS * BW;
    b.partial_items = w.partial_plain + R * (size_t)frw::MSM_FOLD1_THREADS * BW;
    w.s1 = b.partial_items + R * (size_t)b.max_items * BW;
    w.s0 = w.s1 + R * BW;
    w.window_sums = w.s0 + R * BW;
    w.row_start = (unsigned long long *)(w.window_sums + (size_t)frw::WIDE_W * BW);
    w.bin_start = w.row_start + R;
    w.row_count = (uint32_t *)(w.bin_start + frw::WIDE_ALL_BINS);
    w.bin_count = w.row_count + R;
    w.slice_hist = w.bin_count + frw::WIDE_ALL_BINS;
    w.coarse = (uint2 *)(w.slice_hist + (size_t)frw::WIDE_W * frw::WIDE_SLICES * frw::WIDE_BINS);
    w.entries = (uint32_t *)(w.coarse + (size_t)frw::WIDE_W * n);
    w.digits = (int32_t *)w.entries;
    w.end = w.entries + (size_t)frw::WIDE_W * n;
    b.entries = w.entries; b.ones_list = w.end; b.end = w.end;
    return w;
}
template <class F> size_t msm_workspace_per_signature(uint32_t n, bool bare = false, bool wide = false)
{
    if (wide) {
        char *const base0 = (char *)(uintptr_t)4096;
        return ((size_t)((char *)msm_carve_wide<F>(base0, n).end - base0) + 15) & ~(size_t)15;
    }
    const size_t rows = bare ? frw::MSM_W : 1;
    char *const base = (char *)(uintptr_t)4096;
    const size_t bytes = (size_t)((char *)msm_carve<F>(base, rows, n, bare).end - base) + (bare ? (size_t)frw::MSM_W * frw::Grp<F>::BK_WORDS * 4 : 0);
    return (bytes + 15) & ~(size_t)15;
}

struct NmsmBufs {
    uint32_t *slice_hist, *counts, *offsets, *item_first, *items, *item_count, *ones_count, *ones_list, *entries;
    uint32_t *partial_items, *partial_ones, *folded_ones, *bucket_sums;
    uint32_t target, max_items, ones_stride;
    uint32_t n = 0;
    unsigned long long *entry_base = nullptr;
    uint32_t *window_sums = nullptr;
    uint32_t *end = nullptr;
};
template <class F> NmsmBufs nmsm_carve(void *d_workspace, size_t cnt, uint32_t n)
{
    constexpr int BW = frw::Grp<F>::BK_WORDS;
    NmsmBufs b;
    b.target = frw::nmsm_target_items(n); b.max_items = frw::nmsm_max_items(n); b.ones_stride = frw::nmsm_ones_max(n) / 64;
    b.slice_hist = (uint32_t *)d_workspace;
    b.counts = b.slice_hist + cnt * (size_t)frw::nmsm_slices(n) * frw::NMSM_BUCKETS;
    b.offsets = b.counts + cnt * frw::NMSM_BUCKETS;
    b.item_first = b.offsets + cnt * frw::NMSM_BUCKETS;
    b.items = b.item_first + cnt * frw::NMSM_BUCKETS;
    b.item_count = b.items + cnt * (size_t)b.max_items;
    b.ones_count = b.item_count + cnt * 4;
    b.ones_list = b.ones_count + cnt * 4;
    b.entries = b.ones_list + cnt * (size_t)n;
    b.partial_items = b.entries + cnt * (size_t)frw::NMSM_W * n;
    b.partial_items += (4 - ((uintptr_t)b.partial_items >> 2 & 3)) & 3;
    b.partial_ones = b.partial_items + cnt * (size_t)b.max_items * BW;
    b.folded_ones = b.partial_ones + cnt * (size_t)b.ones_stride * BW;
    b.bucket_sums = b.folded_ones + (b.ones_stride > 64 ? cnt * (size_t)64 * BW : 0);
    b.end = b.bucket_sums + cnt * (size_t)frw::NMSM_BUCKETS * BW;
    return b;
}
template <class F> NmsmBufs nmsm_carve_bare(void *d_workspace, size_t tables, uint32_t n, const NmsmBufs *sorted = nullptr)
{
    constexpr int BW = frw::Grp<F>::BK_WORDS;
    constexpr size_t WIN = frw::NMSM_W;
    NmsmBufs b;
    uint32_t *p = (uint32_t *)d_workspace;
    if (sorted) {
        b = *sorted;
    } else {
        b.target = frw::nmsm_target_items(n); b.max_items = frw::nmsm_max_items(n); b.ones_stride = frw::nmsm_ones_max(n) / 64;
        b.n = n;
        b.entry_base = (unsigned long long *)d_workspace;
        b.slice_hist = (uint32_t *)(b.entry_base + WIN);
        b.counts = b.slice_hist + WIN * (size_t)frw::nmsm_slices(n) * frw::NMSM_BUCKETS;
        b.offsets = b.counts + WIN * frw::NMSM_BUCKETS;
        b.item_first = b.offsets + WIN * frw::NMSM_BUCKETS;
        b.items = b.item_first + WIN * frw::NMSM_BUCKETS;
        b.item_count = b.items + WIN * (size_t)b.max_items;
        b.ones_count = b.item_count + WIN * 4;
        p = b.ones_count + 4;
    }
    b.partial_items = p;
    b.partial_ones = b.partial_items + tables * WIN * (size_t)b.max_items * BW;
    b.folded_ones = b.partial_ones + tables * (size_t)b.ones_stride * BW;
    b.bucket_sums = b.folded_ones + tables * (size_t)64 * BW;
    b.window_sums = b.bucket_sums + tables * WIN * (size_t)frw::NMSM_BUCKETS * BW;
    b.end = b.window_sums + tables * WIN * BW;
    if (!sorted) {
        b.ones_list = b.end;
        b.entries = b.ones_list + (size_t)n;
        b.end = b.entries + WIN * (size_t)n;
    }
    return b;
}
template <class F> size_t nmsm_workspace_per_signature(uint32_t n, bool bare = false)
{
    char *const base = (char *)(uintptr_t)4096;
    const NmsmBufs b = bare ? nmsm_carve_bare<F>(base, 1, n) : nmsm_carve<F>(base, 1, n);
    return (((size_t)((char *)b.end - base) + 16) + 15) & ~(size_t)15;
}

template <class F> int msm_load(int device, int group, size_t num_points, const uint64_t *bases, int window_bits, bool bare, frw_msm **out, bool force_wide = false)
{
    if (!out || !bases || num_points == 0 || num_points > (bare ? ((size_t)1 << 31) - 1 : (size_t)1 << (window_bits == 8 ? 25 : 26))) return FRW_E_INVALID_ARG;
    *out = nullptr;
    int ndev = 0;
    if (hipGetDeviceCount(&ndev) != hipSuccess || device < 0 || device >= ndev) return FRW_E_NO_DEVICE;
    hipError_t e = hipSetDevice(device);
    if (e != hipSuccess) return frw::record_hip_error(e, "hipSetDevice");
    frw_msm *m = new (std::nothrow) frw_msm;
    if (!m) return FRW_E_OUT_OF_MEMORY;
    m->device = device;
    m->group = group;
    m->window_bits = window_bits;
    m->bare = bare;
    m->wide = bare && window_bits == 16 && (force_wide || num_points >= msm_wide_from());
    m->table = nullptr;
    m->ones_table = nullptr;
    m->dev.ones_table = nullptr;
    m->dev.n = (uint32_t)num_points;
    void *d_bases = nullptr;
    const size_t table_bytes = (size_t)(bare ? 1 : 256 / window_bits) * num_points * frw::Grp<F>::PT_WORDS * 4, ark_bytes = (size_t)frw::Grp<F>::ARK_WORDS * 4;
    e = hipMalloc(&m->table, table_bytes);
    if (e == hipSuccess) e = hipMalloc(&d_bases, num_points * ark_bytes);
    if (e == hipSuccess) e = hipMemcpy(d_bases, bases, num_points * ark_bytes, hipMemcpyHostToDevice);
    if (e == hipSuccess) {
        hipLaunchKernelGGL(frw::msm_precompute_kernel<F>, dim3((unsigned)((num_points + 63) / 64)), dim3(64), 0, nullptr,
                           (uint32_t)num_points, (const uint32_t *)d_bases, (uint32_t *)m->table, bare ? 256 : window_bits);
        e = hipGetLastError();
    }
    if (e == hipSuccess) e = hipDeviceSynchronize();
    if (d_bases) (void)hipFree(d_bases);
    d_bases = nullptr;
    if (e == hipSuccess && !bare && window_bits == 8 && num_points <= ((size_t)1 << 18)) {
        const size_t entries = (num_points + 7) / 8 * 255;
        e = hipMalloc(&m->ones_table, entries * frw::Grp<F>::PT_WORDS * 4);
        if (e == hipSuccess) {
            hipLaunchKernelGGL(frw::msm_ones_table_kernel<F>, dim3((unsigned)((entries + 63) / 64)), dim3(64), 0, nullptr, (uint32_t)num_points,
                               (const uint32_t *)m->table, (uint32_t *)m->ones_table);
            e = hipGetLastError();
        }
        if (e == hipSuccess) e = hipDeviceSynchronize();
    }
    if (e != hipSuccess) {
        frw_msm_free(m);
        return frw::record_hip_error(e, "frw_msm_load");
    }
    m->dev.table = (const uint32_t *)m->table;
    m->dev.ones_table = (const uint32_t *)m->ones_table;
    *out = m;
    return FRW_OK;
}

template <class F> int fixed_base(int device, size_t count, const uint64_t *scalars, uint64_t *out)
{
    if (count && (!scalars || !out)) return FRW_E_INVALID_ARG;
    if (count == 0) return FRW_OK;
    int ndev = 0;
    if (hipGetDeviceCount(&ndev) != hipSuccess || device < 0 || device >= ndev) return FRW_E_NO_DEVICE;
    hipError_t e = hipSetDevice(device);
    void *d_table = nullptr, *d_sc = nullptr, *d_out = nullptr;
    const size_t ark_bytes = (size_t)frw::Grp<F>::ARK_WORDS * 4;
    if (e == hipSuccess) e = hipMalloc(&d_table, (size_t)frw::FB_WINDOWS * frw::FB_DIGITS * frw::Grp<F>::PT_WORDS * 4);
    if (e == hipSuccess) e = hipMalloc(&d_sc, count * 32);
    if (e == hipSuccess) e = hipMalloc(&d_out, count * ark_bytes);
    if (e == hipSuccess) e = hipMemcpy(d_sc, scalars, count * 32, hipMemcpyHostToDevice);
    if (e == hipSuccess) {
        hipLaunchKernelGGL(frw::fixed_base_table_kernel<F>, dim3(frw::FB_WINDOWS * frw::FB_DIGITS / 64), dim3(64), 0, nullptr, (uint32_t *)d_table);
        hipLaunchKernelGGL(frw::fixed_base_kernel<F>, dim3((unsigned)((count + 63) / 64)), dim3(64), 0, nullptr, count,
                           (const uint32_t *)d_sc, (const uint32_t *)d_table, (uint32_t *)d_out);
        e = hipGetLastError();
    }
    if (e == hipSuccess) e = hipMemcpy(out, d_out, count * ark_bytes, hipMemcpyDeviceToHost);
    for (void *p : {d_table, d_sc, d_out})
        if (p) (void)hipFree(p);
    return e == hipSuccess ? FRW_OK : frw::record_hip_error(e, "frw_fixed_base");
}

template <class F, bool PREFETCH>
hipError_t msm_rows(const frw_msm *m, size_t rows, const uint32_t *sc, size_t stride_words, int montgomery, uint32_t *out, bool xyzz_out,
                    void *d_workspace, hipStream_t st)
{
    const uint32_t n = m->dev.n;
    const bool bare = m->bare;
    const MsmBufs<F> b = msm_carve<F>(d_workspace, rows, n, bare);
    uint32_t *slice_hist = b.buckets;
    const int slices = rows == 1 ? frw::MSM_SLICES_LONE : frw::MSM_SLICES;
    if (rows == 1) slice_hist = b.partial_items;
    const dim3 sgrid((unsigned)slices, (unsigned)rows);
    hipError_t e = hipMemsetAsync(b.ones_count, 0, rows * 16, st);
    if (e != hipSuccess) return e;
    if (bare) {
        hipLaunchKernelGGL(frw::msm_digits_kernel, dim3((n + 255) / 256), dim3(256), 0, st, n, sc, montgomery, b.digits);
        hipLaunchKernelGGL(frw::msm_hist_digits_kernel, sgrid, dim3(1024), 0, st, n, (const int16_t *)b.digits, slice_hist);
    } else {
        hipLaunchKernelGGL(frw::msm_hist_kernel, sgrid, dim3(1024), 0, st, n, sc, stride_words, montgomery, slice_hist, b.ones_count, b.ones_list, 0);
    }
    hipLaunchKernelGGL(frw::msm_slice_offsets_kernel, dim3(frw::MSM_BUCKETS / 256, (unsigned)rows), dim3(256), 0, st, slice_hist, b.counts, slices);
    hipLaunchKernelGGL(frw::msm_scan_kernel, dim3((unsigned)rows), dim3(1024), 0, st, b.counts, b.offsets);
    const uint32_t finer = bare ? 1u : rows <= 2 ? (n > (1u << 18) ? 24u : 4u) : 1u;
    hipLaunchKernelGGL(frw::msm_order_kernel, dim3((unsigned)rows), dim3(1024), 0, st, b.counts, b.offsets, b.order, b.item_first, b.items, b.item_count, finer,
                       b.max_items);
    if (bare) hipLaunchKernelGGL(frw::msm_scatter_digits_kernel, sgrid, dim3(1024), 0, st, n, (const int16_t *)b.digits, b.offsets, slice_hist, b.entries);
    else hipLaunchKernelGGL(frw::msm_scatter_kernel, sgrid, dim3(1024), 0, st, n, sc, stride_words, montgomery, b.offsets, slice_hist, b.entries, 0);
    hipLaunchKernelGGL((frw::msm_bucket_kernel<F, PREFETCH>), dim3(b.max_items / 64, (unsigned)rows), dim3(64), 0, st, m->dev, b.offsets,
                       b.counts, b.items, b.item_count, b.entries, b.partial_items, finer, b.max_items, b.ent_stride, (const unsigned long long *)nullptr);
    hipLaunchKernelGGL(frw::msm_combine_kernel<F>, dim3(frw::MSM_BUCKETS / 64, (unsigned)rows), dim3(64), 0, st, b.offsets, b.counts, b.item_first,
                       b.partial_items, b.buckets, finer, b.max_items);
    const int log_chunk = rows >= 128 ? 6 : rows >= 32 ? 5 : 3;
    const unsigned t1 = (unsigned)frw::MSM_BUCKETS >> log_chunk;
    frw::MsmDev ones_dev = m->dev;
    if (bare) ones_dev.n = 0;
    hipLaunchKernelGGL(frw::msm_ones_kernel<F>, dim3(t1 / 64, (unsigned)rows), dim3(64), 0, st, ones_dev, b.ones_count, b.ones_list, b.partial);
    if (log_chunk == 6) hipLaunchKernelGGL((frw::msm_fold1_kernel<F, 6>), dim3(t1 / 64, (unsigned)rows), dim3(64), 0, st, b.buckets, b.partial, (uint32_t *)nullptr);
    else if (log_chunk == 5) hipLaunchKernelGGL((frw::msm_fold1_kernel<F, 5>), dim3(t1 / 64, (unsigned)rows), dim3(64), 0, st, b.buckets, b.partial, (uint32_t *)nullptr);
    else hipLaunchKernelGGL((frw::msm_fold1_kernel<F, 3>), dim3(t1 / 64, (unsigned)rows), dim3(64), 0, st, b.buckets, b.partial, (uint32_t *)nullptr);
    hipLaunchKernelGGL(frw::msm_fold2_kernel<F>, dim3((unsigned)rows), dim3(frw::MSM_FOLD_THREADS), 0, st, b.partial,
                       (int)(t1 / frw::MSM_FOLD_THREADS), out, xyzz_out ? 1 : 0);
    return hipGetLastError();
}
template <class F, bool PREFETCH>
hipError_t msm_rows_wide(const frw_msm *m, const uint32_t *sc, int montgomery, uint32_t *out, bool xyzz_out, void *d_workspace, hipStream_t st)
{
    constexpr unsigned R = frw::WIDE_ROWS;
    const uint32_t n = m->dev.n;
    const MsmWideBufs<F> w = msm_carve_wide<F>(d_workspace, n);
    const MsmBufs<F> &b = w.rows;
    hipError_t e = hipMemsetAsync(b.ones_count, 0, R * 16, st);
    if (e != hipSuccess) return e;
    const dim3 sgrid(frw::WIDE_SLICES, frw::WIDE_W);
    hipLaunchKernelGGL(frw::msm_wide_digits_kernel, dim3((n + 255) / 256), dim3(256), 0, st, n, sc, montgomery, w.digits);
    hipLaunchKernelGGL(frw::msm_wide_bin_hist_kernel, sgrid, dim3(1024), 0, st, n, (const int32_t *)w.digits, w.slice_hist);
    hipLaunchKernelGGL(frw::msm_wide_bin_offsets_kernel, dim3(1), dim3(1024), 0, st, (uint32_t)frw::WIDE_SLICES, w.slice_hist, w.bin_count, w.bin_start, w.row_count,
                       w.row_start);
    hipLaunchKernelGGL(frw::msm_wide_bin_scatter_kernel, sgrid, dim3(1024), 0, st, n, (const int32_t *)w.digits, (const uint32_t *)w.slice_hist,
                       (const unsigned long long *)w.bin_start, w.coarse);
    uint32_t *part_hist = b.buckets;
    static_assert((size_t)frw::WIDE_ALL_BINS * frw::WIDE_PARTS * frw::WIDE_BIN_BUCKETS <= (size_t)R * frw::MSM_BUCKETS * frw::Grp<F>::BK_WORDS, "the parts' histograms borrow the buckets");
    const dim3 pgrid(frw::WIDE_ALL_BINS * frw::WIDE_PARTS);
    hipLaunchKernelGGL(frw::msm_wide_bucket_hist_kernel, pgrid, dim3(1024), 0, st, (const uint2 *)w.coarse, (const uint32_t *)w.bin_count,
                       (const unsigned long long *)w.bin_start, part_hist);
    hipLaunchKernelGGL(frw::msm_wide_bucket_parts_kernel, dim3(frw::WIDE_ALL_BINS), dim3(1024), 0, st, part_hist, b.counts);
    hipLaunchKernelGGL(frw::msm_scan_kernel, dim3(R), dim3(1024), 0, st, b.counts, b.offsets);
    hipLaunchKernelGGL(frw::msm_order_kernel, dim3(R), dim3(1024), 0, st, b.counts, b.offsets, b.order, b.item_first, b.items, b.item_count, 1u, b.max_items);
    hipLaunchKernelGGL(frw::msm_wide_bucket_scatter_kernel, pgrid, dim3(1024), 0, st, (const uint2 *)w.coarse, (const uint32_t *)w.bin_count,
                       (const unsigned long long *)w.bin_start, (const uint32_t *)b.offsets, (const uint32_t *)part_hist, (const unsigned long long *)w.row_start,
                       w.entries);
    hipLaunchKernelGGL((frw::msm_bucket_kernel<F, PREFETCH>), dim3(b.max_items / 64, R), dim3(64), 0, st, m->dev, b.offsets, b.counts, b.items, b.item_count,
                       w.entries, b.partial_items, 1u, b.max_items, (size_t)0, (const unsigned long long *)w.row_start);
    hipLaunchKernelGGL(frw::msm_combine_kernel<F>, dim3(frw::MSM_BUCKETS / 64, R), dim3(64), 0, st, b.offsets, b.counts, b.item_first, b.partial_items,
                       b.buckets, 1u, b.max_items);
    constexpr int LOG_CHUNK = 6;
    const unsigned t1 = (unsigned)frw::MSM_BUCKETS >> LOG_CHUNK;
    frw::MsmDev ones_dev = m->dev;
    ones_dev.n = 0;
    hipLaunchKernelGGL(frw::msm_ones_kernel<F>, dim3(t1 / 64, R), dim3(64), 0, st, ones_dev, b.ones_count, b.ones_list, b.partial);
    hipLaunchKernelGGL((frw::msm_fold1_kernel<F, LOG_CHUNK>), dim3(t1 / 64, R), dim3(64), 0, st, b.buckets, b.partial, w.partial_plain);
    hipLaunchKernelGGL(frw::msm_fold2_kernel<F>, dim3(R), dim3(frw::MSM_FOLD_THREADS), 0, st, b.partial, (int)(t1 / frw::MSM_FOLD_THREADS), w.s1, 1);
    hipLaunchKernelGGL(frw::msm_fold2_kernel<F>, dim3(R), dim3(frw::MSM_FOLD_THREADS), 0, st, w.partial_plain, (int)(t1 / frw::MSM_FOLD_THREADS), w.s0, 1);
    hipLaunchKernelGGL(frw::msm_wide_window_kernel<F>, dim3(frw::WIDE_W), dim3(64), 0, st, (const uint32_t *)w.s1, (const uint32_t *)w.s0, w.window_sums);
    hipLaunchKernelGGL(frw::msm_horner_kernel<F>, dim3(1), dim3(64), 0, st, (const uint32_t *)w.window_sums, (int)frw::WIDE_W, (int)frw::WIDE_C, out, xyzz_out ? 1 : 0);
    return hipGetLastError();
}
template <class F, bool PREFETCH>
int msm_run(const frw_msm *m, size_t batch, const uint64_t *d_scalars, size_t scalar_stride, int montgomery, uint64_t *d_out,
            void *d_workspace, size_t workspace_bytes, hipStream_t st, bool xyzz_out = false)
{
    const uint32_t n = m->dev.n;
    const size_t per = msm_workspace_per_signature<F>(n, m->bare, m->wide);
    size_t chunk = workspace_bytes / per;
    if (chunk == 0 || ((uintptr_t)d_workspace & 15)) return FRW_E_INVALID_ARG;
    if (chunk > 32768) chunk = 32768;
    constexpr int BW = frw::Grp<F>::BK_WORDS;
    hipError_t e = hipSetDevice(m->device);
    if (m->wide) {
        for (size_t sig = 0; e == hipSuccess && sig < batch; sig++)
            e = msm_rows_wide<F, PREFETCH>(m, (const uint32_t *)(d_scalars + sig * scalar_stride * 4), montgomery,
                                           (uint32_t *)d_out + sig * (xyzz_out ? BW : frw::Grp<F>::ARK_WORDS), xyzz_out, d_workspace, st);
        return e == hipSuccess ? FRW_OK : frw::record_hip_error(e, "frw_msm_dev");
    }
    if (m->bare) {
        uint32_t *window_sums = (uint32_t *)((char *)d_workspace + per) - (size_t)frw::MSM_W * BW;
        for (size_t sig = 0; e == hipSuccess && sig < batch; sig++) {
            e = msm_rows<F, PREFETCH>(m, frw::MSM_W, (const uint32_t *)(d_scalars + sig * scalar_stride * 4), 0, montgomery, window_sums, true, d_workspace, st);
            if (e != hipSuccess) break;
            hipLaunchKernelGGL(frw::msm_horner_kernel<F>, dim3(1), dim3(64), 0, st, window_sums, frw::MSM_W, frw::MSM_C,
                               (uint32_t *)d_out + sig * (xyzz_out ? BW : frw::Grp<F>::ARK_WORDS), xyzz_out ? 1 : 0);
            e = hipGetLastError();
        }
        return e == hipSuccess ? FRW_OK : frw::record_hip_error(e, "frw_msm_dev");
    }
    for (size_t lo = 0; e == hipSuccess && lo < batch; lo += chunk) {
        const size_t cnt = batch - lo < chunk ? batch - lo : chunk;
        e = msm_rows<F, PREFETCH>(m, cnt, (const uint32_t *)(d_scalars + lo * scalar_stride * 4), scalar_stride * 8, montgomery,
                                  (uint32_t *)d_out + lo * (xyzz_out ? BW : frw::Grp<F>::ARK_WORDS), xyzz_out, d_workspace, st);
    }
    return e == hipSuccess ? FRW_OK : frw::record_hip_error(e, "frw_msm_dev");
}
hipError_t nmsm_sort(const NmsmBufs &b, uint32_t n, size_t cnt, const uint32_t *sc, size_t stride_words, int montgomery, bool ones_as_mask, hipStream_t st)
{
    const uint32_t slices = frw::nmsm_slices(n);
    const dim3 sgrid(slices, (unsigned)cnt);
    hipError_t e = hipMemsetAsync(b.ones_count, 0, cnt * 4, st);
    if (e == hipSuccess && ones_as_mask) e = hipMemsetAsync(b.ones_list, 0, cnt * (size_t)n * 4, st);
    if (e != hipSuccess) return e;
    hipLaunchKernelGGL(frw::nmsm_hist_kernel, sgrid, dim3(1024), 0, st, n, sc, stride_words, montgomery, b.slice_hist, b.ones_count, b.ones_list,
                       ones_as_mask ? 1 : 0);
    hipLaunchKernelGGL(frw::nmsm_plan_kernel, dim3((unsigned)cnt), dim3(frw::NMSM_BUCKETS), 0, st, b.slice_hist, b.counts, b.offsets, b.item_first, b.items,
                       b.item_count, b.target, b.max_items, slices);
    hipLaunchKernelGGL(frw::nmsm_scatter_kernel, sgrid, dim3(1024), 0, st, n, sc, stride_words, montgomery, b.offsets, b.slice_hist, b.entries);
    return hipGetLastError();
}
hipError_t nmsm_sort_bare(const NmsmBufs &b, uint32_t n, const uint32_t *sc, int montgomery, hipStream_t st, const uint32_t *index = nullptr)
{
    const uint32_t slices = frw::nmsm_slices(n);
    hipError_t e = hipMemsetAsync(b.ones_count, 0, 16, st);
    if (e != hipSuccess) return e;
    hipLaunchKernelGGL(frw::nmsm_hist_bare_kernel, dim3(slices), dim3(1024), 0, st, n, sc, montgomery, b.slice_hist, b.ones_count, b.ones_list, index);
    hipLaunchKernelGGL(frw::nmsm_plan_kernel, dim3(frw::NMSM_W), dim3(frw::NMSM_BUCKETS), 0, st, b.slice_hist, b.counts, b.offsets, b.item_first, b.items,
                       b.item_count, b.target, b.max_items, slices);
    hipLaunchKernelGGL(frw::nmsm_entry_base_kernel, dim3(1), dim3(64), 0, st, b.counts, b.offsets, b.entry_base);
    hipLaunchKernelGGL(frw::nmsm_scatter_bare_kernel, dim3(slices), dim3(1024), 0, st, n, sc, montgomery, b.offsets, b.slice_hist, b.entry_base, b.entries,
                       index);
    return hipGetLastError();
}
template <class F, bool PREFETCH>
hipError_t nmsm_accumulate(const frw_msm *const *ms, int tables, const NmsmBufs &sorted, const NmsmBufs &own, size_t cnt, uint32_t *d_out, bool ones_as_mask,
                           hipStream_t st, bool xyzz_out = false, bool ones_elsewhere = false, hipStream_t ones_stream = nullptr, hipEvent_t ones_done = nullptr)
{
    if (!ones_elsewhere) ones_stream = st;
    const uint32_t n = ms[0]->dev.n;
    frw::NmsmTables dev;
    dev.n = n; dev.sigs = (uint32_t)cnt;
    for (int t = 0; t < 3; t++) {
        const frw_msm *m = ms[t < tables ? t : 0];
        dev.table[t] = m->dev.table;
        dev.ones_table[t] = ones_as_mask ? m->dev.ones_table : nullptr;
    }
    const unsigned rows = (unsigned)(cnt * (size_t)tables);
    typedef typename frw::BulkPolicy<F>::type FB;
    static const bool g2_prefetch = std::getenv("FRW_G2_PREFETCH") != nullptr;
    int ones_threads = 256;
    while (ones_threads < (int)frw::nmsm_ones_max(n) && (size_t)ones_threads * rows < 65536) ones_threads <<= 1;
    hipLaunchKernelGGL(frw::nmsm_ones_kernel<FB>, dim3((unsigned)ones_threads / 64, rows), dim3(64), 0, ones_stream, dev, sorted.ones_count, sorted.ones_list,
                       own.partial_ones, own.ones_stride, 1u);
    const uint32_t *ones_for_finish = own.partial_ones;
    uint32_t ones_groups = (uint32_t)ones_threads / 64, ones_finish_stride = own.ones_stride;
    if (ones_groups > 64) {
        hipLaunchKernelGGL(frw::nmsm_ones_fold_kernel<FB>, dim3(64, rows), dim3(64), 0, ones_stream, own.partial_ones, ones_groups, own.ones_stride, own.folded_ones);
        ones_for_finish = own.folded_ones;
        ones_groups = 64;
        ones_finish_stride = 64;
    }
    if (ones_elsewhere) {
        const hipError_t e = hipEventRecord(ones_done, ones_stream);
        if (e != hipSuccess) return e;
    }
    if (PREFETCH || (FB::LANES > 1 && g2_prefetch))
        hipLaunchKernelGGL((frw::nmsm_bucket_kernel<FB, true>), dim3((sorted.max_items * FB::LANES + 63) / 64, rows), dim3(64), 0, st, dev,
                           sorted.offsets, sorted.counts, sorted.items, sorted.item_count, sorted.entries, own.partial_items, sorted.target, sorted.max_items,
                           (const unsigned long long *)nullptr);
    else
        hipLaunchKernelGGL((frw::nmsm_bucket_kernel<FB, false>), dim3((sorted.max_items * FB::LANES + 63) / 64, rows), dim3(64), 0, st, dev,
                           sorted.offsets, sorted.counts, sorted.items, sorted.item_count, sorted.entries, own.partial_items, sorted.target, sorted.max_items,
                           (const unsigned long long *)nullptr);
    const bool combine = cnt <= 16;
    if (combine)
        hipLaunchKernelGGL(frw::nmsm_combine_kernel<FB>, dim3(frw::NMSM_BUCKETS, rows), dim3(64), 0, st, sorted.counts, sorted.offsets, sorted.item_first,
                           own.partial_items, own.bucket_sums, sorted.target, sorted.max_items, (uint32_t)cnt);
    if (ones_elsewhere) {
        const hipError_t e = hipStreamWaitEvent(st, ones_done, 0);
        if (e != hipSuccess) return e;
    }
    hipLaunchKernelGGL(frw::nmsm_finish_kernel<FB>, dim3(rows), dim3(64), 0, st, sorted.counts, sorted.offsets, sorted.item_first, own.partial_items,
                       combine ? own.bucket_sums : (uint32_t *)nullptr, ones_for_finish, (int)ones_groups, ones_finish_stride, sorted.target, sorted.max_items,
                       d_out, xyzz_out ? 1 : 0, (uint32_t)cnt, 0);
    return hipGetLastError();
}
template <class F, bool PREFETCH>
hipError_t nmsm_accumulate_bare(const frw_msm *const *ms, int tables, const NmsmBufs &b, uint32_t *d_out, hipStream_t st, bool xyzz_out, uint32_t out_step = 1)
{
    const uint32_t n = b.n;
    frw::NmsmTables dev;
    dev.n = n; dev.sigs = frw::NMSM_W;
    for (int t = 0; t < 3; t++) {
        dev.table[t] = ms[t < tables ? t : 0]->dev.table;
        dev.ones_table[t] = nullptr;
    }
    const unsigned rows = (unsigned)tables * frw::NMSM_W;
    typedef typename frw::BulkPolicy<F>::type FB;
    static const bool g2_prefetch = std::getenv("FRW_G2_PREFETCH") != nullptr;
    const uint32_t ones_threads = frw::nmsm_ones_max(n);
    hipLaunchKernelGGL(frw::nmsm_ones_kernel<FB>, dim3(ones_threads / 64, (unsigned)tables), dim3(64), 0, st, dev, b.ones_count, b.ones_list, b.partial_ones,
                       b.ones_stride, (uint32_t)frw::NMSM_W);
    const uint32_t *ones_for_finish = b.partial_ones;
    uint32_t ones_groups = ones_threads / 64, ones_finish_stride = b.ones_stride;
    if (ones_groups > 64) {
        hipLaunchKernelGGL(frw::nmsm_ones_fold_kernel<FB>, dim3(64, (unsigned)tables), dim3(64), 0, st, b.partial_ones, ones_groups, b.ones_stride, b.folded_ones);
        ones_for_finish = b.folded_ones;
        ones_groups = 64;
        ones_finish_stride = 64;
    }
    if (PREFETCH || (FB::LANES > 1 && g2_prefetch))
        hipLaunchKernelGGL((frw::nmsm_bucket_kernel<FB, true>), dim3((b.max_items * FB::LANES + 63) / 64, rows), dim3(64), 0, st, dev,
                           b.offsets, b.counts, b.items, b.item_count, b.entries, b.partial_items, b.target, b.max_items, (const unsigned long long *)b.entry_base);
    else
        hipLaunchKernelGGL((frw::nmsm_bucket_kernel<FB, false>), dim3((b.max_items * FB::LANES + 63) / 64, rows), dim3(64), 0, st, dev,
                           b.offsets, b.counts, b.items, b.item_count, b.entries, b.partial_items, b.target, b.max_items, (const unsigned long long *)b.entry_base);
    hipLaunchKernelGGL(frw::nmsm_combine_kernel<FB>, dim3(frw::NMSM_BUCKETS, rows), dim3(64), 0, st, b.counts, b.offsets, b.item_first,
                       b.partial_items, b.bucket_sums, b.target, b.max_items, (uint32_t)frw::NMSM_W);
    hipLaunchKernelGGL(frw::nmsm_finish_kernel<FB>, dim3(rows), dim3(64), 0, st, b.counts, b.offsets, b.item_first, b.partial_items,
                       b.bucket_sums, ones_for_finish, (int)ones_groups, ones_finish_stride, b.target, b.max_items,
                       b.window_sums, 1, (uint32_t)frw::NMSM_W, 1);
    hipLaunchKernelGGL(frw::msm_horner_kernel<FB>, dim3((unsigned)tables), dim3(64), 0, st, b.window_sums, frw::NMSM_W, frw::NMSM_C, d_out, xyzz_out ? 1 : 0,
                       out_step);
    return hipGetLastError();
}
template <class F, bool PREFETCH>
int nmsm_run(const frw_msm *m, size_t batch, const uint64_t *d_scalars, size_t scalar_stride, int montgomery, uint64_t *d_out,
             void *d_workspace, size_t workspace_bytes, hipStream_t st)
{
    const uint32_t n = m->dev.n;
    const size_t per = nmsm_workspace_per_signature<F>(n, m->bare);
    size_t chunk = workspace_bytes / per;
    if (chunk == 0 || ((uintptr_t)d_workspace & 15)) return FRW_E_INVALID_ARG;
    if (chunk > 32768) chunk = 32768;
    hipError_t e = hipSetDevice(m->device);
    if (m->bare) {
        const NmsmBufs b = nmsm_carve_bare<F>(d_workspace, 1, n);
        for (size_t sig = 0; e == hipSuccess && sig < batch; sig++) {
            e = nmsm_sort_bare(b, n, (const uint32_t *)(d_scalars + sig * scalar_stride * 4), montgomery, st);
            if (e == hipSuccess) e = nmsm_accumulate_bare<F, PREFETCH>(&m, 1, b, (uint32_t *)(d_out + sig * (frw::Grp<F>::ARK_WORDS / 2)), st, false);
        }
        return e == hipSuccess ? FRW_OK : frw::record_hip_error(e, "frw_msm_dev");
    }
    for (size_t lo = 0; e == hipSuccess && lo < batch; lo += chunk) {
        const size_t cnt = batch - lo < chunk ? batch - lo : chunk;
        const NmsmBufs b = nmsm_carve<F>(d_workspace, cnt, n);
        e = nmsm_sort(b, n, cnt, (const uint32_t *)(d_scalars + lo * scalar_stride * 4), scalar_stride * 8, montgomery, m->ones_table != nullptr, st);
        if (e == hipSuccess)
            e = nmsm_accumulate<F, PREFETCH>(&m, 1, b, b, cnt, (uint32_t *)(d_out + lo * (frw::Grp<F>::ARK_WORDS / 2)), m->ones_table != nullptr, st);
    }
    return e == hipSuccess ? FRW_OK : frw::record_hip_error(e, "frw_msm_dev");
}
}

extern "C" void frw_msm_free(frw_msm *m)
{
    if (!m) return;
    (void)hipSetDevice(m->device);
    if (m->table) (void)hipFree(m->table);
    if (m->ones_table) (void)hipFree(m->ones_table);
    delete m;
}

extern "C" int frw_msm_g1_load(int device, size_t num_points, const uint64_t *bases, frw_msm **out)
{
    return msm_load<FqField>(device, 1, num_points, bases, 16, false, out);
}
extern "C" int frw_msm_g1_load_narrow(int device, size_t num_points, const uint64_t *bases, frw_msm **out)
{
    return msm_load<FqField>(device, 1, num_points, bases, 8, false, out);
}
extern "C" int frw_msm_g2_load_narrow(int device, size_t num_points, const uint64_t *bases, frw_msm **out)
{
    return msm_load<Fq2Field>(device, 2, num_points, bases, 8, false, out);
}
extern "C" int frw_msm_g2_load(int device, size_t num_points, const uint64_t *bases, frw_msm **out)
{
    return msm_load<Fq2Field>(device, 2, num_points, bases, 16, false, out);
}
extern "C" int frw_msm_g1_load_bare(int device, size_t num_points, const uint64_t *bases, int narrow, frw_msm **out)
{
    if (narrow < 0 || narrow > 2) return FRW_E_INVALID_ARG;
    return msm_load<FqField>(device, 1, num_points, bases, narrow == 1 ? 8 : 16, true, out, narrow == 2);
}
extern "C" int frw_msm_g2_load_bare(int device, size_t num_points, const uint64_t *bases, int narrow, frw_msm **out)
{
    if (narrow < 0 || narrow > 2) return FRW_E_INVALID_ARG;
    return msm_load<Fq2Field>(device, 2, num_points, bases, narrow == 1 ? 8 : 16, true, out, narrow == 2);
}
extern "C" int frw_g1_fixed_base(int device, size_t count, const uint64_t *scalars, uint64_t *out)
{
    return fixed_base<FqField>(device, count, scalars, out);
}
extern "C" int frw_g2_fixed_base(int device, size_t count, const uint64_t *scalars, uint64_t *out)
{
    return fixed_base<Fq2Field>(device, count, scalars, out);
}

extern "C" int frw_msm_info(const frw_msm *m, frw_msm_info_t *out)
{
    if (!m || !out) return FRW_E_INVALID_ARG;
    const bool g2 = m->group == 2;
    out->num_points = m->dev.n;
    const bool narrow = m->window_bits == 8;
    out->window_bits = m->wide ? frw::WIDE_C : m->window_bits;
    out->num_windows = m->wide ? frw::WIDE_W : 256 / m->window_bits;
    out->table_bytes = (uint64_t)(m->bare ? 1 : out->num_windows) * m->dev.n * (g2 ? frw::Grp<Fq2Field>::PT_WORDS : frw::Grp<FqField>::PT_WORDS) * 4;
    if (m->ones_table) out->table_bytes += (uint64_t)((m->dev.n + 7) / 8) * 255 * (g2 ? frw::Grp<Fq2Field>::PT_WORDS : frw::Grp<FqField>::PT_WORDS) * 4;
    const uint32_t n = m->dev.n;
    const bool bare = m->bare;
    out->workspace_bytes_per_signature = narrow ? (g2 ? nmsm_workspace_per_signature<Fq2Field>(n, bare) : nmsm_workspace_per_signature<FqField>(n, bare))
                                                : (g2 ? msm_workspace_per_signature<Fq2Field>(n, bare, m->wide) : msm_workspace_per_signature<FqField>(n, bare, m->wide));
    return FRW_OK;
}

extern "C" int frw_msm_g1_dev(const frw_msm *m, size_t batch, const uint64_t *d_scalars, size_t scalar_stride, int montgomery,
                              uint64_t *d_out, void *d_workspace, size_t workspace_bytes, void *stream)
{
    if (!m || m->group != 1 || (batch && (!d_scalars || !d_out || !d_workspace)) || scalar_stride < m->dev.n) return FRW_E_INVALID_ARG;
    if (batch == 0) return FRW_OK;
    if (m->window_bits == 8) return nmsm_run<FqField, true>(m, batch, d_scalars, scalar_stride, montgomery, d_out, d_workspace, workspace_bytes, (hipStream_t)stream);
    return msm_run<FqField, true>(m, batch, d_scalars, scalar_stride, montgomery, d_out, d_workspace, workspace_bytes, (hipStream_t)stream);
}
extern "C" int frw_msm_g2_dev(const frw_msm *m, size_t batch, const uint64_t *d_scalars, size_t scalar_stride, int montgomery,
                              uint64_t *d_out, void *d_workspace, size_t workspace_bytes, void *stream)
{
    if (!m || m->group != 2 || (batch && (!d_scalars || !d_out || !d_workspace)) || scalar_stride < m->dev.n) return FRW_E_INVALID_ARG;
    if (batch == 0) return FRW_OK;
    if (m->window_bits == 8) return nmsm_run<Fq2Field, false>(m, batch, d_scalars, scalar_stride, montgomery, d_out, d_workspace, workspace_bytes, (hipStream_t)stream);
    return msm_run<Fq2Field, false>(m, batch, d_scalars, scalar_stride, montgomery, d_out, d_workspace, workspace_bytes, (hipStream_t)stream);
}

extern "C" int frw_groth16_msm_h_dev(const frw_msm *m, size_t batch, const uint64_t *d_h, size_t domain_size, uint64_t *d_out,
                                     void *d_workspace, size_t workspace_bytes, void *stream)
{
    if (!m || (size_t)m->dev.n + 1 != domain_size) return FRW_E_INVALID_ARG;
    return frw_msm_g1_dev(m, batch, d_h, domain_size, 1, d_out, d_workspace, workspace_bytes, stream);
}

namespace frw {
__device__ const uint32_t FR_TO_MONT[NL29] = {0x1e538d9eu, 0x19e99103u, 0x13b31eccu, 0x04e2d5e4u, 0x181dac62u, 0x115f1ba1u,
                                              0x1e414fbbu, 0x11b3009cu, 0x00013fecu};
__global__ __launch_bounds__(64) void groth16_tails_kernel(size_t batch, const uint32_t *__restrict__ rs ,
                                                           uint32_t *__restrict__ zext, size_t stride_words, size_t nv)
{
    const size_t sig = (size_t)blockIdx.x * 64 + threadIdx.x;
    if (sig >= batch) return;
    uint32_t *dst = zext + sig * stride_words + nv * 8;
    constexpr uint32_t one[8] = FRW_R32;
    Fr8 o;
#pragma unroll
    for (int k = 0; k < 8; k++) o.l[k] = one[k];
    fr_store(dst, o);
    F29 c;
#pragma unroll
    for (int k = 0; k < NL29; k++) c.l[k] = FR_TO_MONT[k];
    for (int j = 0; j < 2; j++)
        fr_store(dst + 8 * (j + 1), f29_pack(f29_canonical(f29_mul(f29_unpack(fr_load(rs + (sig * 2 + j) * 8)), c))));
}
__global__ __launch_bounds__(64) void groth16_split_kernel(size_t count, const uint64_t *__restrict__ rs , uint64_t *__restrict__ out )
{
    const size_t i = (size_t)blockIdx.x * 64 + threadIdx.x;
    if (i >= count) return;
    const uint64_t R[4] = {0xffffffff00000001ULL, 0x53bda402fffe5bfeULL, 0x3339d80809a1d805ULL, 0x73eda753299d7d48ULL};
    const uint64_t L0 = 0x00000000ffffffffULL, L1 = 0xac45a4010001a402ULL;
    uint64_t k[4] = {rs[i * 4], rs[i * 4 + 1], rs[i * 4 + 2], rs[i * 4 + 3]};
    for (int round = 0; round < 2; round++) {
        bool ge = true;
        for (int j = 3; j >= 0; j--)
            if (k[j] != R[j]) { ge = k[j] > R[j]; break; }
        if (!ge) break;
        uint64_t borrow = 0;
        for (int j = 0; j < 4; j++) {
            const uint64_t d = k[j] - R[j], d2 = d - borrow;
            borrow = (k[j] < R[j]) | (d < borrow);
            k[j] = d2;
        }
    }
    uint64_t r0 = 0, r1 = 0, q0 = 0, q1 = 0;
    for (int bit = 255; bit >= 0; bit--) {
        const uint64_t top = r1 >> 63;
        r1 = (r1 << 1) | (r0 >> 63);
        r0 = (r0 << 1) | ((k[bit >> 6] >> (bit & 63)) & 1ULL);
        q1 = (q1 << 1) | (q0 >> 63);
        q0 <<= 1;
        if (top || r1 > L1 || (r1 == L1 && r0 >= L0)) {
            const uint64_t b = r0 < L0;
            r0 -= L0;
            r1 = r1 - L1 - b;
            q0 |= 1ULL;
        }
    }
    out[i * 4] = r0; out[i * 4 + 1] = r1; out[i * 4 + 2] = q0; out[i * 4 + 3] = q1;
}
struct QuadLaneExec {
    uint32_t *lds;
    uint32_t lane;
    static __device__ __forceinline__ void fence()
    {
        __builtin_amdgcn_fence(__ATOMIC_RELEASE, "workgroup");
        __builtin_amdgcn_wave_barrier();
        __builtin_amdgcn_fence(__ATOMIC_ACQUIRE, "workgroup");
    }
    static __device__ __forceinline__ uint32_t from_lane0(uint32_t x)
    {
        return (uint32_t)__builtin_amdgcn_mov_dpp((int)x, 0x00 , 0xf, 0xf, true);
    }
    template <const quad::Step &S> __device__ __forceinline__ void step(uint32_t qx, uint32_t qy)
    {
        Fq29 a;
        const Fq29 r = quad::compute<S>(lds, lane, qx, qy, a);
        quad::store<S>(lds, lane, r);
        fence();
    }
    template <const quad::Step &S> __device__ __forceinline__ void step_test(uint32_t qx, uint32_t qy, bool &pz)
    {
        Fq29 a;
        const Fq29 r = quad::compute<S>(lds, lane, qx, qy, a);
        quad::store<S>(lds, lane, r);
        fence();
        pz = from_lane0(fq_is_zero(a) ? 1u : 0u) != 0;
    }
    __device__ __forceinline__ bool degenerate(uint32_t qx, uint32_t qy)
    {
        uint32_t inf = 0;
        if (lane == 0) inf = quad::add_degenerate(lds, qx, qy) ? 1u : 0u;
        fence();
        return from_lane0(inf) != 0;
    }
};
__global__ __launch_bounds__(4) void groth16_scale_quad_kernel(size_t batch, const uint32_t *__restrict__ split ,
                                                               const uint32_t *__restrict__ pts ,
                                                               uint32_t *__restrict__ out )
{
    __builtin_amdgcn_s_setprio(2);
    typedef FqField F;
    constexpr int BW = Grp<F>::BK_WORDS;
    __shared__ __attribute__((aligned(16))) uint32_t file[quad::NSLOTS * quad::SLOT_WORDS];
    const size_t slot = blockIdx.x;
    const uint32_t lane = threadIdx.x;
    if (slot >= 2 * batch) return;
    const size_t sig = slot < batch ? slot : slot - batch;
    const int which = slot < batch ? 1 : 0;
    if (pts[slot * BW + 4 * F::WORDS] != 0) {
        if (lane == 0) store_bucket<F>(out + slot * BW, pt_identity<F>());
        return;
    }
    if (lane == 0) quad::setup(file, load_bucket<F>(pts + slot * BW));
    QuadLaneExec::fence();
    const uint32_t *k = split + (sig * 2 + which) * 8;
    uint32_t k0[4], k1[4];
#pragma unroll
    for (int i = 0; i < 4; i++) { k0[i] = k[i]; k1[i] = k[4 + i]; }
    QuadLaneExec ex{file, lane};
    const bool inf = quad::scalar_mul(ex, k0, k1);
    if (lane == 0) store_bucket<F>(out + slot * BW, inf ? pt_identity<F>() : quad::running_point(file, false));
}
__global__ __launch_bounds__(64) void groth16_finish_kernel(size_t batch, const uint32_t *__restrict__ a_pts, const uint32_t *__restrict__ sa_pts,
                                                            const uint32_t *__restrict__ rb1_pts, const uint32_t *__restrict__ l_pts,
                                                            const uint32_t *__restrict__ h_pts ,
                                                            const uint32_t *__restrict__ b2_pts ,
                                                            uint32_t *__restrict__ proofs )
{
    __builtin_amdgcn_s_setprio(2);
    typedef FqField F;
    constexpr int BW = Grp<F>::BK_WORDS;
    const size_t t = (size_t)blockIdx.x * 64 + threadIdx.x, sig = t >> 1;
    const bool holds_a = (t & 1) != 0;
    if (sig >= batch) return;
    XyzzT<F> acc = load_bucket<F>((holds_a ? a_pts : l_pts) + sig * BW);
#pragma nounroll
    for (int j = 0; j < 3; j++) {
        const uint32_t *p = j == 0 ? h_pts : j == 1 ? sa_pts : rb1_pts;
        if (!holds_a) acc = pt_add(acc, load_bucket<F>(p + sig * BW));
    }
    uint32_t *o = proofs + sig * 96;
    if (!holds_a)
        for (int k = 0; k < 48; k++) o[24 + k] = b2_pts[sig * 48 + k];
    store_ark_point<F>(o + (holds_a ? 0 : 72), pt_to_affine(acc));
}
__global__ __launch_bounds__(64) void groth16_partial_kernel(const uint32_t *__restrict__ g1_pts ,
                                                             const uint32_t *__restrict__ b2_ark , uint32_t *__restrict__ out )
{
    const uint32_t t = threadIdx.x;
    if (t < 4) store_ark_point<FqField>(out + t * 24, pt_to_affine(load_bucket<FqField>(g1_pts + t * Grp<FqField>::BK_WORDS)));
    else if (t < 4 + 48) out[96 + (t - 4)] = b2_ark[t - 4];
}
__global__ __launch_bounds__(64) void groth16_combine_kernel(uint32_t world, const uint32_t *__restrict__ partials ,
                                                             uint32_t *__restrict__ g1_pts , uint32_t *__restrict__ b2_ark )
{
    const uint32_t t = threadIdx.x;
    if (t < 4) {
        XyzzT<FqField> acc = pt_identity<FqField>();
        for (uint32_t r = 0; r < world; r++) acc = pt_add_affine(acc, load_ark_point<FqField>(partials + (size_t)r * 144 + t * 24));
        store_bucket<FqField>(g1_pts + t * Grp<FqField>::BK_WORDS, acc);
    } else if (t == 4) {
        XyzzT<Fq2Field> acc = pt_identity<Fq2Field>();
        for (uint32_t r = 0; r < world; r++) acc = pt_add_affine(acc, load_ark_point<Fq2Field>(partials + (size_t)r * 144 + 96));
        store_ark_point<Fq2Field>(b2_ark, pt_to_affine(acc));
    }
}
}

struct frw_groth16_pk {
    int device;
    uint64_t num_instance, num_witness, domain_size;
    frw_msm *h, *a, *b1, *l, *b2;
    bool bare = false;
    uint32_t rank = 0, world = 1;
    uint64_t z_lo = 0, z_hi = 0, h_lo = 0, h_hi = 0;
    uint32_t *b_index = nullptr;
    uint32_t b_rows = 0;
    hipStream_t main, side[3];
    hipEvent_t fork, sorted, ones_done, join[4];
    std::mutex enqueue;
};

extern "C" void frw_groth16_pk_free(frw_groth16_pk *pk)
{
    if (!pk) return;
    for (frw_msm *m : {pk->h, pk->a, pk->b1, pk->l, pk->b2}) frw_msm_free(m);
    (void)hipSetDevice(pk->device);
    if (pk->b_index) (void)hipFree(pk->b_index);
    for (int i = 0; i < 4; i++) {
        if (i < 3 && pk->side[i]) (void)hipStreamDestroy(pk->side[i]);
        if (pk->join[i]) (void)hipEventDestroy(pk->join[i]);
// ... 646 lines not shown
```

Baseline: 1.333 million.

## Run G2 MSM kernels with branch-free incomplete formulas and flagged complete fallback

```diff
diff --git a/falcon-r1cs_amd/csrc/frw_fq29.h b/falcon-r1cs_amd/csrc/frw_fq29.h
--- a/falcon-r1cs_amd/csrc/frw_fq29.h
+++ b/falcon-r1cs_amd/csrc/frw_fq29.h
@@ -708,6 +708,77 @@
     r.inf = false;
     return r;
 }
+__host__ __device__ __forceinline__ Fq29 el_select(bool a_, const Fq29 &a, const Fq29 &b)
+{
+    Fq29 r;
+#pragma unroll
+    for (int i = 0; i < NLQ; i++) r.l[i] = a_ ? a.l[i] : b.l[i];
+    return r;
+}
+__host__ __device__ __forceinline__ Fq2_29 el_select(bool a_, const Fq2_29 &a, const Fq2_29 &b)
+{
+    Fq2_29 r;
+    r.c0 = el_select(a_, a.c0, b.c0);
+    r.c1 = el_select(a_, a.c1, b.c1);
+    return r;
+}
+#if defined(__HIPCC__)
+__device__ __forceinline__ Fq2Half el_select(bool a_, const Fq2Half &a, const Fq2Half &b) { Fq2Half r; r.v = el_select(a_, a.v, b.v); return r; }
+#endif
+template <class F> __host__ __device__ __forceinline__ XyzzT<F> pt_select(bool a_, const XyzzT<F> &a, const XyzzT<F> &b)
+{
+    XyzzT<F> r;
+    r.x = el_select(a_, a.x, b.x); r.y = el_select(a_, a.y, b.y); r.zz = el_select(a_, a.zz, b.zz); r.zzz = el_select(a_, a.zzz, b.zzz);
+    r.inf = a_ ? a.inf : b.inf;
+    return r;
+}
+template <class F> __host__ __device__ __forceinline__ XyzzT<F> pt_add_affine_fast(const XyzzT<F> &p, const AffineT<F> &q, bool &equal_x)
+{
+    const auto u2 = F::mul(q.x, p.zz), s2 = F::mul(q.y, p.zzz);
+    const auto pp_ = F::template sub<F::K_X>(u2, p.x);
+    const auto rr = F::template sub<F::K_Y>(s2, p.y);
+    const bool z = F::is_zero(pp_);
+    equal_x |= z && !p.inf && !q.inf;
+    const auto pp = F::sqr(pp_), ppp = F::mul(pp_, pp), qq = F::mul(p.x, pp);
+    XyzzT<F> r;
+    r.x = F::template sub<F::K_2MUL>(F::template sub<F::K_MUL>(F::sqr(rr), ppp), F::add(qq, qq));
+    r.y = F::template mul_sub<F::K_Y>(rr, F::template sub<F::K_X>(qq, r.x), p.y, ppp);
+    r.zz = F::mul(p.zz, pp);
+    r.zzz = F::mul(p.zzz, ppp);
+    r.inf = false;
+    return pt_select(q.inf, p, pt_select(p.inf, pt_from_affine(q), r));
+}
+template <class F> __host__ __device__ __forceinline__ XyzzT<F> pt_add_fast(const XyzzT<F> &p, const XyzzT<F> &q, bool &equal_x)
+{
+    const auto u1 = F::mul(p.x, q.zz), u2 = F::mul(q.x, p.zz), s1 = F::mul(p.y, q.zzz), s2 = F::mul(q.y, p.zzz);
+    const auto pp_ = F::template sub<F::K_MUL>(u2, u1), rr = F::template sub<F::K_MUL>(s2, s1);
+    const bool z = F::is_zero(pp_);
+    equal_x |= z && !p.inf && !q.inf;
+    const auto pp = F::sqr(pp_), ppp = F::mul(pp_, pp), qq = F::mul(u1, pp);
+    XyzzT<F> r;
+    r.x = F::template sub<F::K_2MUL>(F::template sub<F::K_MUL>(F::sqr(rr), ppp), F::add(qq, qq));
+    r.y = F::template mul_sub<F::K_MUL>(rr, F::template sub<F::K_X>(qq, r.x), s1, ppp);
+    r.zz = F::mul(F::mul(p.zz, q.zz), pp);
+    r.zzz = F::mul(F::mul(p.zzz, q.zzz), ppp);
+    r.inf = false;
+    return pt_select(q.inf, p, pt_select(p.inf, q, r));
+}
+template <class F> __host__ __device__ __forceinline__ XyzzT<F> pt_double_fast(const XyzzT<F> &p)
+{
+    const auto u = F::add(p.y, p.y);
+    const auto v = F::sqr(u), w = F::mul(u, v);
+    const auto s = F::mul(p.x, v);
+    const auto xx = F::sqr(p.x);
+    const auto m = F::add(F::add(xx, xx), xx);
+    XyzzT<F> r;
+    r.x = F::template sub<F::K_2MUL>(F::sqr(m), F::add(s, s));
+    r.y = F::template mul_sub<F::K_MUL>(m, F::template sub<F::K_X>(s, r.x), w, p.y);
+    r.zz = F::mul(v, p.zz);
+    r.zzz = F::mul(w, p.zzz);
+    r.inf = false;
+    return pt_select(p.inf, p, r);
+}
+
 template <class F> __host__ __device__ inline AffineT<F> pt_to_affine(const XyzzT<F> &p)
 {
     AffineT<F> r;
diff --git a/falcon-r1cs_amd/csrc/frw_msm.hip b/falcon-r1cs_amd/csrc/frw_msm.hip
--- a/falcon-r1cs_amd/csrc/frw_msm.hip
+++ b/falcon-r1cs_amd/csrc/frw_msm.hip
@@ -684,22 +684,57 @@
     store_bucket<F>(partial_items + (sig * (size_t)max_items + it) * (size_t)Grp<F>::BK_WORDS, acc);
 }
 
-template <class F>
-__global__ __launch_bounds__(64) void msm_horner_kernel(const uint32_t *__restrict__ sums, int windows, int window_bits,
+template <class F, bool COMPLETE> struct SumOps {
+    bool equal_x = false;
+    __device__ __forceinline__ XyzzT<F> add_affine(const XyzzT<F> &p, const AffineT<F> &q)
+    {
+        if constexpr (COMPLETE) return pt_add_affine(p, q);
+        else return pt_add_affine_fast(p, q, equal_x);
+    }
+    __device__ __forceinline__ XyzzT<F> add(const XyzzT<F> &p, const XyzzT<F> &q)
+    {
+        if constexpr (COMPLETE) return pt_add(p, q);
+        else return pt_add_fast(p, q, equal_x);
+    }
+    __device__ __forceinline__ XyzzT<F> dbl(const XyzzT<F> &p)
+    {
+        if constexpr (COMPLETE) return pt_double(p);
+        else return pt_double_fast(p);
+    }
+    __device__ __forceinline__ static bool skip(const uint32_t *flags)
+    {
+        return COMPLETE && flags && !flags[blockIdx.y * (size_t)gridDim.x + blockIdx.x];
+    }
+    __device__ __forceinline__ void report(uint32_t *flags) const
+    {
+        if constexpr (!COMPLETE) {
+            const bool any = __any(equal_x) != 0;
+            if (threadIdx.x == 0) flags[blockIdx.y * (size_t)gridDim.x + blockIdx.x] = any ? 1u : 0u;
+        }
+    }
+};
+template <class F, bool COMPLETE> struct SumWaves { static constexpr int value = F::LANES > 1 && COMPLETE ? 1 : 2; };
+template <class F, bool COMPLETE = true>
+__global__ __launch_bounds__(64, (SumWaves<F, COMPLETE>::value)) void msm_horner_kernel(const uint32_t *__restrict__ sums, int windows, int window_bits,
                                                         uint32_t *__restrict__ out , int xyzz_out,
-                                                        uint32_t out_step = 1 )
-{
+                                                        uint32_t out_step = 1 , uint32_t *__restrict__ flags = nullptr)
+{
+    typedef SumOps<F, COMPLETE> Ops;
+    if (Ops::skip(flags)) return;
     __builtin_amdgcn_s_setprio(2);
     constexpr int BW = Grp<F>::BK_WORDS;
-    if (threadIdx.x >= (unsigned)F::LANES) return;
-    const uint32_t *src = sums + (size_t)blockIdx.x * windows * BW;
-    XyzzT<F> acc = load_bucket<F>(src + (size_t)(windows - 1) * BW);
-    for (int j = windows - 2; j >= 0; j--) {
-        for (int k = 0; k < window_bits; k++) acc = pt_double(acc);
-        acc = pt_add(acc, load_bucket<F>(src + (size_t)j * BW));
-    }
-    if (xyzz_out) store_bucket<F>(out + (size_t)blockIdx.x * out_step * BW, acc);
-    else store_ark_point<F>(out + (size_t)blockIdx.x * Grp<F>::ARK_WORDS, pt_to_affine(acc));
+    Ops ops;
+    if (threadIdx.x < (unsigned)F::LANES) {
+        const uint32_t *src = sums + (size_t)blockIdx.x * windows * BW;
+        XyzzT<F> acc = load_bucket<F>(src + (size_t)(windows - 1) * BW);
+        for (int j = windows - 2; j >= 0; j--) {
+            for (int k = 0; k < window_bits; k++) acc = ops.dbl(acc);
+            acc = ops.add(acc, load_bucket<F>(src + (size_t)j * BW));
+        }
+        if (xyzz_out) store_bucket<F>(out + (size_t)blockIdx.x * out_step * BW, acc);
+        else store_ark_point<F>(out + (size_t)blockIdx.x * Grp<F>::ARK_WORDS, pt_to_affine(acc));
+    }
+    ops.report(flags);
 }
 template <int PT_WORDS_>
 __global__ __launch_bounds__(1024) void live_rows_kernel(const uint32_t *__restrict__ rows, uint32_t n, uint32_t *__restrict__ block_counts ,
@@ -1032,53 +1067,62 @@
         }
     }
 }
-template <class F, bool PREFETCH>
-__global__ __launch_bounds__(64, F::LANES > 1 ? 1 : 2) void nmsm_bucket_kernel(NmsmTables tables, const uint32_t *__restrict__ offsets, const uint32_t *__restrict__ counts,
+template <class F, bool PREFETCH, bool COMPLETE = true>
+__global__ __launch_bounds__(64, (SumWaves<F, COMPLETE>::value)) void nmsm_bucket_kernel(NmsmTables tables, const uint32_t *__restrict__ offsets, const uint32_t *__restrict__ counts,
                                                             const uint32_t *__restrict__ items, const uint32_t *__restrict__ item_count,
                                                             const uint32_t *__restrict__ entries, uint32_t *__restrict__ partial_items,
                                                             uint32_t target, uint32_t max_items,
-                                                            const unsigned long long *__restrict__ entry_base )
-{
+                                                            const unsigned long long *__restrict__ entry_base ,
+                                                            uint32_t *__restrict__ flags = nullptr)
+{
+    typedef SumOps<F, COMPLETE> Ops;
+    if (Ops::skip(flags)) return;
     __builtin_amdgcn_s_setprio(2);
     constexpr int PW = Grp<F>::PT_WORDS;
     const size_t slot = blockIdx.y;
     size_t sig;
     const MsmDev m = tables.of(blockIdx.y, sig);
     const uint32_t it = (blockIdx.x * 64 + threadIdx.x) / F::LANES;
-    if (it >= item_count[sig]) return;
-    const uint32_t item = items[sig * (size_t)max_items + it], b = item & (NMSM_BUCKETS - 1), part = item >> 8;
-    const uint32_t c = counts[sig * NMSM_BUCKETS + b];
-    const uint32_t total = offsets[sig * NMSM_BUCKETS + NMSM_BUCKETS - 1] + counts[sig * NMSM_BUCKETS + NMSM_BUCKETS - 1], split = nmsm_split_of(total, target);
-    const uint32_t k = c <= split ? 1u : (c + split - 1) / split;
-    const uint32_t lo = (uint32_t)((uint64_t)c * part / k), cnt = (uint32_t)((uint64_t)c * (part + 1) / k) - lo;
-    const uint32_t *ent = entries + (entry_base ? (size_t)entry_base[sig] : sig * (size_t)NMSM_W * m.n) + offsets[sig * NMSM_BUCKETS + b] + lo;
-    XyzzT<F> acc = pt_identity<F>();
-    if (PREFETCH) {
-        uint32_t e = cnt ? ent[0] : 0u;
-        AffineT<F> p = load_row<F>(m.table + (size_t)(e & 0x7fffffffu) * PW);
-        for (uint32_t j = 0; j < cnt; j++) {
-            const uint32_t e_next = j + 1 < cnt ? ent[j + 1] : e;
-            const AffineT<F> p_next = load_row<F>(m.table + (size_t)(e_next & 0x7fffffffu) * PW);
-            if (e >> 31) p.y = F::template neg<Grp<F>::K_AFFINE_Y>(p.y);
-            acc = pt_add_affine(acc, p);
-            e = e_next;
-            p = p_next;
-        }
-    } else {
-        for (uint32_t j = 0; j < cnt; j++) {
-            const uint32_t e = ent[j];
+    Ops ops;
+    if (it < item_count[sig]) {
+        const uint32_t item = items[sig * (size_t)max_items + it], b = item & (NMSM_BUCKETS - 1), part = item >> 8;
+        const uint32_t c = counts[sig * NMSM_BUCKETS + b];
+        const uint32_t total = offsets[sig * NMSM_BUCKETS + NMSM_BUCKETS - 1] + counts[sig * NMSM_BUCKETS + NMSM_BUCKETS - 1], split = nmsm_split_of(total, target);
+        const uint32_t k = c <= split ? 1u : (c + split - 1) / split;
+        const uint32_t lo = (uint32_t)((uint64_t)c * part / k), cnt = (uint32_t)((uint64_t)c * (part + 1) / k) - lo;
+        const uint32_t *ent = entries + (entry_base ? (size_t)entry_base[sig] : sig * (size_t)NMSM_W * m.n) + offsets[sig * NMSM_BUCKETS + b] + lo;
+        XyzzT<F> acc = pt_identity<F>();
+        if (PREFETCH) {
+            uint32_t e = cnt ? ent[0] : 0u;
             AffineT<F> p = load_row<F>(m.table + (size_t)(e & 0x7fffffffu) * PW);
-            if (e >> 31) p.y = F::template neg<Grp<F>::K_AFFINE_Y>(p.y);
-            acc = pt_add_affine(acc, p);
-        }
-    }
-    store_bucket<F>(partial_items + (slot * (size_t)max_items + it) * (size_t)Grp<F>::BK_WORDS, acc);
-}
-template <class F>
-__global__ __launch_bounds__(64, F::LANES > 1 ? 1 : 2) void nmsm_ones_kernel(NmsmTables tables, const uint32_t *__restrict__ ones_count, const uint32_t *__restrict__ ones_list,
+            for (uint32_t j = 0; j < cnt; j++) {
+                const uint32_t e_next = j + 1 < cnt ? ent[j + 1] : e;
+                const AffineT<F> p_next = load_row<F>(m.table + (size_t)(e_next & 0x7fffffffu) * PW);
+                if (e >> 31) p.y = F::template neg<Grp<F>::K_AFFINE_Y>(p.y);
+                acc = ops.add_affine(acc, p);
+                e = e_next;
+                p = p_next;
+            }
+        } else {
+            for (uint32_t j = 0; j < cnt; j++) {
+                const uint32_t e = ent[j];
+                AffineT<F> p = load_row<F>(m.table + (size_t)(e & 0x7fffffffu) * PW);
+                if (e >> 31) p.y = F::template neg<Grp<F>::K_AFFINE_Y>(p.y);
+                acc = ops.add_affine(acc, p);
+            }
+        }
+        store_bucket<F>(partial_items + (slot * (size_t)max_items + it) * (size_t)Grp<F>::BK_WORDS, acc);
+    }
+    ops.report(flags);
+}
+template <class F, bool COMPLETE = true>
+__global__ __launch_bounds__(64, (SumWaves<F, COMPLETE>::value)) void nmsm_ones_kernel(NmsmTables tables, const uint32_t *__restrict__ ones_count, const uint32_t *__restrict__ ones_list,
                                                           uint32_t *__restrict__ partial_ones , uint32_t groups_stride,
-                                                          uint32_t row_step )
-{
+                                                          uint32_t row_step ,
+                                                          uint32_t *__restrict__ flags = nullptr)
+{
+    typedef SumOps<F, COMPLETE> Ops;
+    if (Ops::skip(flags)) return;
     __builtin_amdgcn_s_setprio(2);
     constexpr int SLOT = 4 * F::WORDS + 1, PER = 64 / F::LANES;
     __shared__ uint32_t lds[32 * SLOT];
@@ -1087,55 +1131,63 @@
     const MsmDev m = tables.of(blockIdx.y * row_step, sig);
     const uint32_t nthreads = gridDim.x * PER, t = blockIdx.x * PER + threadIdx.x / F::LANES;
     const uint32_t *list = ones_list + sig * m.n;
+    Ops ops;
     XyzzT<F> acc = pt_identity<F>();
     if (m.ones_table) {
         const uint32_t groups = (m.n + 7) / 8;
         for (uint32_t g = t; g < groups; g += nthreads) {
             const uint32_t byte = (list[g >> 2] >> (8 * (g & 3))) & 0xffu;
-            if (byte) acc = pt_add_affine(acc, load_row<F>(m.ones_table + ((size_t)g * 255 + (byte - 1)) * Grp<F>::PT_WORDS));
+            if (byte) acc = ops.add_affine(acc, load_row<F>(m.ones_table + ((size_t)g * 255 + (byte - 1)) * Grp<F>::PT_WORDS));
         }
     } else {
         const uint32_t cnt = ones_count[sig];
         for (uint32_t k = t; k < cnt; k += nthreads)
-            acc = pt_add_affine(acc, load_row<F>(m.table + (size_t)list[k] * Grp<F>::PT_WORDS));
+            acc = ops.add_affine(acc, load_row<F>(m.table + (size_t)list[k] * Grp<F>::PT_WORDS));
     }
     const int lane = threadIdx.x / F::LANES;
     for (int stride = PER / 2; stride >= 1; stride >>= 1) {
         if (lane >= stride && lane < 2 * stride) store_bucket<F>(lds + (lane - stride) * SLOT, acc);
         __syncthreads();
-        if (lane < stride) acc = pt_add(acc, load_bucket<F>(lds + lane * SLOT));
+        if (lane < stride) acc = ops.add(acc, load_bucket<F>(lds + lane * SLOT));
         __syncthreads();
     }
     if (lane == 0) store_bucket<F>(partial_ones + (slot * (size_t)groups_stride + blockIdx.x) * (size_t)Grp<F>::BK_WORDS, acc);
+    ops.report(flags);
 }
 template <class F> struct BulkPolicy { typedef F type; };
 template <> struct BulkPolicy<Fq2Field> { typedef Fq2PairField type; };
-template <class F>
-__global__ __launch_bounds__(64, F::LANES > 1 ? 1 : 2) void nmsm_ones_fold_kernel(const uint32_t *__restrict__ partial_ones, uint32_t groups, uint32_t groups_stride,
-                                                               uint32_t *__restrict__ folded )
-{
+template <class F, bool COMPLETE = true>
+__global__ __launch_bounds__(64, (SumWaves<F, COMPLETE>::value)) void nmsm_ones_fold_kernel(const uint32_t *__restrict__ partial_ones, uint32_t groups, uint32_t groups_stride,
+                                                               uint32_t *__restrict__ folded , uint32_t *__restrict__ flags = nullptr)
+{
+    typedef SumOps<F, COMPLETE> Ops;
+    if (Ops::skip(flags)) return;
     __builtin_amdgcn_s_setprio(2);
     constexpr int SLOT = 4 * F::WORDS + 1, BW = Grp<F>::BK_WORDS, PER = 64 / F::LANES;
     __shared__ uint32_t lds[32 * SLOT];
     const size_t sig = blockIdx.y;
     const uint32_t g = blockIdx.x, lane = threadIdx.x / F::LANES;
     const uint32_t *src = partial_ones + sig * (size_t)groups_stride * BW;
+    Ops ops;
     XyzzT<F> acc = pt_identity<F>();
-    for (uint32_t k = g + 64 * lane; k < groups; k += 64 * PER) acc = pt_add(acc, load_bucket<F>(src + (size_t)k * BW));
+    for (uint32_t k = g + 64 * lane; k < groups; k += 64 * PER) acc = ops.add(acc, load_bucket<F>(src + (size_t)k * BW));
     for (int stride = PER / 2; stride >= 1; stride >>= 1) {
         if ((int)lane >= stride && (int)lane < 2 * stride) store_bucket<F>(lds + (lane - stride) * SLOT, acc);
         __syncthreads();
-        if ((int)lane < stride) acc = pt_add(acc, load_bucket<F>(lds + lane * SLOT));
+        if ((int)lane < stride) acc = ops.add(acc, load_bucket<F>(lds + lane * SLOT));
         __syncthreads();
     }
     if (lane == 0) store_bucket<F>(folded + (sig * 64 + g) * (size_t)BW, acc);
-}
-template <class F>
-__global__ __launch_bounds__(64, F::LANES > 1 ? 1 : 2) void nmsm_combine_kernel(const uint32_t *__restrict__ counts, const uint32_t *__restrict__ offsets,
+    ops.report(flags);
+}
+template <class F, bool COMPLETE = true>
+__global__ __launch_bounds__(64, (SumWaves<F, COMPLETE>::value)) void nmsm_combine_kernel(const uint32_t *__restrict__ counts, const uint32_t *__restrict__ offsets,
                                                              const uint32_t *__restrict__ item_first, const uint32_t *__restrict__ partial_items,
                                                              uint32_t *__restrict__ buckets , uint32_t target, uint32_t max_items,
-                                                             uint32_t sigs)
-{
+                                                             uint32_t sigs, uint32_t *__restrict__ flags = nullptr)
+{
+    typedef SumOps<F, COMPLETE> Ops;
+    if (Ops::skip(flags)) return;
     __builtin_amdgcn_s_setprio(2);
     constexpr int SLOT = 4 * F::WORDS + 1, BW = Grp<F>::BK_WORDS, PER = 64 / F::LANES;
     __shared__ uint32_t lds[32 * SLOT];
@@ -1145,26 +1197,31 @@
     const uint32_t total = offsets[sig * NMSM_BUCKETS + NMSM_BUCKETS - 1] + counts[sig * NMSM_BUCKETS + NMSM_BUCKETS - 1], split = nmsm_split_of(total, target);
     const uint32_t k = c <= split ? 1u : (c + split - 1) / split;
     const uint32_t *src = partial_items + (slot * (size_t)max_items + item_first[sig * NMSM_BUCKETS + b]) * (size_t)BW;
+    Ops ops;
     XyzzT<F> acc = pt_identity<F>();
-    for (uint32_t j = lane; j < k; j += PER) acc = pt_add(acc, load_bucket<F>(src + (size_t)j * BW));
+    for (uint32_t j = lane; j < k; j += PER) acc = ops.add(acc, load_bucket<F>(src + (size_t)j * BW));
     for (int stride = PER / 2; stride >= 1; stride >>= 1) {
         if ((int)lane >= stride && (int)lane < 2 * stride) store_bucket<F>(lds + (lane - stride) * SLOT, acc);
         __syncthreads();
-        if ((int)lane < stride) acc = pt_add(acc, load_bucket<F>(lds + lane * SLOT));
+        if ((int)lane < stride) acc = ops.add(acc, load_bucket<F>(lds + lane * SLOT));
         __syncthreads();
     }
     if (lane == 0) store_bucket<F>(buckets + (slot * NMSM_BUCKETS + b) * (size_t)BW, acc);
-}
-
-template <class F>
-__global__ __launch_bounds__(64) void nmsm_finish_kernel(const uint32_t *__restrict__ counts, const uint32_t *__restrict__ offsets,
+    ops.report(flags);
+}
+
+template <class F, bool COMPLETE = true>
+__global__ __launch_bounds__(64, (SumWaves<F, COMPLETE>::value)) void nmsm_finish_kernel(const uint32_t *__restrict__ counts, const uint32_t *__restrict__ offsets,
                                                          const uint32_t *__restrict__ item_first, const uint32_t *__restrict__ partial_items,
                                                          const uint32_t *__restrict__ buckets ,
                                                          const uint32_t *__restrict__ partial_ones ,
                                                          int ones_groups, uint32_t ones_stride, uint32_t target, uint32_t max_items,
                                                          uint32_t *__restrict__ out , int xyzz_out,
-                                                         uint32_t sigs, int ones_window0 )
-{
+                                                         uint32_t sigs, int ones_window0 ,
+                                                         uint32_t *__restrict__ flags = nullptr)
+{
+    typedef SumOps<F, COMPLETE> Ops;
+    if (Ops::skip(flags)) return;
     __builtin_amdgcn_s_setprio(2);
     constexpr int SLOT = 4 * F::WORDS + 1, BW = Grp<F>::BK_WORDS, PER = 64 / F::LANES, NB = NMSM_BUCKETS / PER;
     constexpr int LOG_PER = PER == 64 ? 6 : 5, LOG_NB = NB == 2 ? 1 : 2;
@@ -1198,6 +1255,7 @@
     const int ones_steps = (ones_groups + PER - 1) / PER;
     const uint32_t at_local = phase0, at_reload = at_local + (NB - 1) + 1, at_scan = at_reload + 1, at_weight = at_scan + LOG_PER,
                    at_final = at_weight + LOG_NB, at_ones = at_final + 1, at_tree = at_ones + ones_steps, steps = at_tree + LOG_PER;
+    Ops ops;
     XyzzT<F> sum = pt_identity<F>();
     for (uint32_t step = 0; step < steps; step++) {
         int store_slot = -1;
@@ -1244,13 +1302,14 @@
         if (store_slot >= 0) store_bucket<F>(lds + store_slot * SLOT, sum);
         __syncthreads();
         if (reset) sum = pt_identity<F>();
-        if (add) sum = pt_add(sum, load_bucket<F>(p));
+        if (add) sum = ops.add(sum, load_bucket<F>(p));
         __syncthreads();
     }
     if (i == 0) {
         if (xyzz_out) store_bucket<F>(out + slot * BW, sum);
         else store_ark_point<F>(out + slot * Grp<F>::ARK_WORDS, pt_to_affine(sum));
     }
+    ops.report(flags);
 }
 
 constexpr int FB_WINDOWS = 32, FB_DIGITS = 256;
@@ -1458,8 +1517,14 @@
     uint32_t n = 0;
     unsigned long long *entry_base = nullptr;
     uint32_t *window_sums = nullptr;
+    uint32_t *flags = nullptr;
     uint32_t *end = nullptr;
 };
+template <class F> constexpr size_t nmsm_flag_words(uint32_t max_items, uint32_t ones_stride, size_t rows, size_t tables)
+{
+    return frw::BulkPolicy<F>::type::LANES == 1 ? 0
+         : ((((size_t)max_items * frw::BulkPolicy<F>::type::LANES + 63) / 64 + ones_stride + 64 + frw::NMSM_BUCKETS + 1) * rows + tables + 3) & ~(size_t)3;
+}
 template <class F> NmsmBufs nmsm_carve(void *d_workspace, size_t cnt, uint32_t n)
 {
     constexpr int BW = frw::Grp<F>::BK_WORDS;
@@ -1479,7 +1544,8 @@
     b.partial_ones = b.partial_items + cnt * (size_t)b.max_items * BW;
     b.folded_ones = b.partial_ones + cnt * (size_t)b.ones_stride * BW;
     b.bucket_sums = b.folded_ones + (b.ones_stride > 64 ? cnt * (size_t)64 * BW : 0);
-    b.end = b.bucket_sums + cnt * (size_t)frw::NMSM_BUCKETS * BW;
+    b.flags = b.bucket_sums + cnt * (size_t)frw::NMSM_BUCKETS * BW;
+    b.end = b.flags + nmsm_flag_words<F>(b.max_items, b.ones_stride, cnt, 0);
     return b;
 }
 template <class F> NmsmBufs nmsm_carve_bare(void *d_workspace, size_t tables, uint32_t n, const NmsmBufs *sorted = nullptr)
@@ -1508,7 +1574,8 @@
     b.folded_ones = b.partial_ones + tables * (size_t)b.ones_stride * BW;
     b.bucket_sums = b.folded_ones + tables * (size_t)64 * BW;
     b.window_sums = b.bucket_sums + tables * WIN * (size_t)frw::NMSM_BUCKETS * BW;
-    b.end = b.window_sums + tables * WIN * BW;
+    b.flags = b.window_sums + tables * WIN * BW;
+    b.end = b.flags + nmsm_flag_words<F>(b.max_items, b.ones_stride, tables * WIN, tables);
     if (!sorted) {
         b.ones_list = b.end;
         b.entries = b.ones_list + (size_t)n;
@@ -1747,6 +1814,16 @@
                        index);
     return hipGetLastError();
 }
+template <class FB> struct NmsmFlags {
+    uint32_t *next;
+    uint32_t *take(dim3 grid)
+    {
+        if (FB::LANES == 1) return nullptr;
+        uint32_t *f = next;
+        next += (size_t)grid.x * grid.y;
+        return f;
+    }
+};
 template <class F, bool PREFETCH>
 hipError_t nmsm_accumulate(const frw_msm *const *ms, int tables, const NmsmBufs &sorted, const NmsmBufs &own, size_t cnt, uint32_t *d_out, bool ones_as_mask,
                            hipStream_t st, bool xyzz_out = false, bool ones_elsewhere = false, hipStream_t ones_stream = nullptr, hipEvent_t ones_done = nullptr)
@@ -1762,15 +1839,23 @@
     }
     const unsigned rows = (unsigned)(cnt * (size_t)tables);
     typedef typename frw::BulkPolicy<F>::type FB;
-    static const bool g2_prefetch = std::getenv("FRW_G2_PREFETCH") != nullptr;
+    constexpr bool TWO = FB::LANES > 1;
+    NmsmFlags<FB> fl{own.flags};
     int ones_threads = 256;
     while (ones_threads < (int)frw::nmsm_ones_max(n) && (size_t)ones_threads * rows < 65536) ones_threads <<= 1;
-    hipLaunchKernelGGL(frw::nmsm_ones_kernel<FB>, dim3((unsigned)ones_threads / 64, rows), dim3(64), 0, ones_stream, dev, sorted.ones_count, sorted.ones_list,
-                       own.partial_ones, own.ones_stride, 1u);
+    const dim3 g_ones((unsigned)ones_threads / 64, rows);
+    uint32_t *f = fl.take(g_ones);
+    if constexpr (TWO)
+        hipLaunchKernelGGL((frw::nmsm_ones_kernel<FB, false>), g_ones, dim3(64), 0, ones_stream, dev, sorted.ones_count, sorted.ones_list, own.partial_ones, own.ones_stride, 1u, f);
+    hipLaunchKernelGGL((frw::nmsm_ones_kernel<FB, true>), g_ones, dim3(64), 0, ones_stream, dev, sorted.ones_count, sorted.ones_list, own.partial_ones, own.ones_stride, 1u, f);
     const uint32_t *ones_for_finish = own.partial_ones;
     uint32_t ones_groups = (uint32_t)ones_threads / 64, ones_finish_stride = own.ones_stride;
     if (ones_groups > 64) {
-        hipLaunchKernelGGL(frw::nmsm_ones_fold_kernel<FB>, dim3(64, rows), dim3(64), 0, ones_stream, own.partial_ones, ones_groups, own.ones_stride, own.folded_ones);
+        const dim3 g_fold(64, rows);
+        f = fl.take(g_fold);
+        if constexpr (TWO)
+            hipLaunchKernelGGL((frw::nmsm_ones_fold_kernel<FB, false>), g_fold, dim3(64), 0, ones_stream, own.partial_ones, ones_groups, own.ones_stride, own.folded_ones, f);
+        hipLaunchKernelGGL((frw::nmsm_ones_fold_kernel<FB, true>), g_fold, dim3(64), 0, ones_stream, own.partial_ones, ones_groups, own.ones_stride, own.folded_ones, f);
         ones_for_finish = own.folded_ones;
         ones_groups = 64;
         ones_finish_stride = 64;
@@ -1779,25 +1864,36 @@
         const hipError_t e = hipEventRecord(ones_done, ones_stream);
         if (e != hipSuccess) return e;
     }
-    if (PREFETCH || (FB::LANES > 1 && g2_prefetch))
-        hipLaunchKernelGGL((frw::nmsm_bucket_kernel<FB, true>), dim3((sorted.max_items * FB::LANES + 63) / 64, rows), dim3(64), 0, st, dev,
-                           sorted.offsets, sorted.counts, sorted.items, sorted.item_count, sorted.entries, own.partial_items, sorted.target, sorted.max_items,
-                           (const unsigned long long *)nullptr);
-    else
-        hipLaunchKernelGGL((frw::nmsm_bucket_kernel<FB, false>), dim3((sorted.max_items * FB::LANES + 63) / 64, rows), dim3(64), 0, st, dev,
-                           sorted.offsets, sorted.counts, sorted.items, sorted.item_count, sorted.entries, own.partial_items, sorted.target, sorted.max_items,
-                           (const unsigned long long *)nullptr);
+    const dim3 g_bucket((sorted.max_items * FB::LANES + 63) / 64, rows);
+    f = fl.take(g_bucket);
+    if constexpr (TWO)
+        hipLaunchKernelGGL((frw::nmsm_bucket_kernel<FB, false, false>), g_bucket, dim3(64), 0, st, dev, sorted.offsets, sorted.counts, sorted.items,
+                           sorted.item_count, sorted.entries, own.partial_items, sorted.target, sorted.max_items, (const unsigned long long *)nullptr, f);
+    hipLaunchKernelGGL((frw::nmsm_bucket_kernel<FB, PREFETCH && !TWO, true>), g_bucket, dim3(64), 0, st, dev, sorted.offsets, sorted.counts, sorted.items,
+                       sorted.item_count, sorted.entries, own.partial_items, sorted.target, sorted.max_items, (const unsigned long long *)nullptr, f);
     const bool combine = cnt <= 16;
-    if (combine)
-        hipLaunchKernelGGL(frw::nmsm_combine_kernel<FB>, dim3(frw::NMSM_BUCKETS, rows), dim3(64), 0, st, sorted.counts, sorted.offsets, sorted.item_first,
-                           own.partial_items, own.bucket_sums, sorted.target, sorted.max_items, (uint32_t)cnt);
+    if (combine) {
+        const dim3 g_comb(frw::NMSM_BUCKETS, rows);
+        f = fl.take(g_comb);
+        if constexpr (TWO)
+            hipLaunchKernelGGL((frw::nmsm_combine_kernel<FB, false>), g_comb, dim3(64), 0, st, sorted.counts, sorted.offsets, sorted.item_first,
+                               own.partial_items, own.bucket_sums, sorted.target, sorted.max_items, (uint32_t)cnt, f);
+        hipLaunchKernelGGL((frw::nmsm_combine_kernel<FB, true>), g_comb, dim3(64), 0, st, sorted.counts, sorted.offsets, sorted.item_first,
+                           own.partial_items, own.bucket_sums, sorted.target, sorted.max_items, (uint32_t)cnt, f);
+    }
     if (ones_elsewhere) {
         const hipError_t e = hipStreamWaitEvent(st, ones_done, 0);
         if (e != hipSuccess) return e;
     }
-    hipLaunchKernelGGL(frw::nmsm_finish_kernel<FB>, dim3(rows), dim3(64), 0, st, sorted.counts, sorted.offsets, sorted.item_first, own.partial_items,
+    const dim3 g_fin(rows);
+    f = fl.take(g_fin);
+    if constexpr (TWO)
+        hipLaunchKernelGGL((frw::nmsm_finish_kernel<FB, false>), g_fin, dim3(64), 0, st, sorted.counts, sorted.offsets, sorted.item_first, own.partial_items,
+                           combine ? own.bucket_sums : (uint32_t *)nullptr, ones_for_finish, (int)ones_groups, ones_finish_stride, sorted.target, sorted.max_items,
+                           d_out, xyzz_out ? 1 : 0, (uint32_t)cnt, 0, f);
+    hipLaunchKernelGGL((frw::nmsm_finish_kernel<FB, true>), g_fin, dim3(64), 0, st, sorted.counts, sorted.offsets, sorted.item_first, own.partial_items,
                        combine ? own.bucket_sums : (uint32_t *)nullptr, ones_for_finish, (int)ones_groups, ones_finish_stride, sorted.target, sorted.max_items,
-                       d_out, xyzz_out ? 1 : 0, (uint32_t)cnt, 0);
+                       d_out, xyzz_out ? 1 : 0, (uint32_t)cnt, 0, f);
     return hipGetLastError();
 }
 template <class F, bool PREFETCH>
@@ -1812,31 +1908,52 @@
     }
     const unsigned rows = (unsigned)tables * frw::NMSM_W;
     typedef typename frw::BulkPolicy<F>::type FB;
-    static const bool g2_prefetch = std::getenv("FRW_G2_PREFETCH") != nullptr;
+    constexpr bool TWO = FB::LANES > 1;
+    NmsmFlags<FB> fl{b.flags};
     const uint32_t ones_threads = frw::nmsm_ones_max(n);
-    hipLaunchKernelGGL(frw::nmsm_ones_kernel<FB>, dim3(ones_threads / 64, (unsigned)tables), dim3(64), 0, st, dev, b.ones_count, b.ones_list, b.partial_ones,
-                       b.ones_stride, (uint32_t)frw::NMSM_W);
+    const dim3 g_ones(ones_threads / 64, (unsigned)tables);
+    uint32_t *f = fl.take(g_ones);
+    if constexpr (TWO)
+        hipLaunchKernelGGL((frw::nmsm_ones_kernel<FB, false>), g_ones, dim3(64), 0, st, dev, b.ones_count, b.ones_list, b.partial_ones, b.ones_stride, (uint32_t)frw::NMSM_W, f);
+    hipLaunchKernelGGL((frw::nmsm_ones_kernel<FB, true>), g_ones, dim3(64), 0, st, dev, b.ones_count, b.ones_list, b.partial_ones, b.ones_stride, (uint32_t)frw::NMSM_W, f);
     const uint32_t *ones_for_finish = b.partial_ones;
     uint32_t ones_groups = ones_threads / 64, ones_finish_stride = b.ones_stride;
     if (ones_groups > 64) {
-        hipLaunchKernelGGL(frw::nmsm_ones_fold_kernel<FB>, dim3(64, (unsigned)tables), dim3(64), 0, st, b.partial_ones, ones_groups, b.ones_stride, b.folded_ones);
+        const dim3 g_fold(64, (unsigned)tables);
+        f = fl.take(g_fold);
+        if constexpr (TWO)
+            hipLaunchKernelGGL((frw::nmsm_ones_fold_kernel<FB, false>), g_fold, dim3(64), 0, st, b.partial_ones, ones_groups, b.ones_stride, b.folded_ones, f);
+        hipLaunchKernelGGL((frw::nmsm_ones_fold_kernel<FB, true>), g_fold, dim3(64), 0, st, b.partial_ones, ones_groups, b.ones_stride, b.folded_ones, f);
         ones_for_finish = b.folded_ones;
         ones_groups = 64;
         ones_finish_stride = 64;
     }
-    if (PREFETCH || (FB::LANES > 1 && g2_prefetch))
-        hipLaunchKernelGGL((frw::nmsm_bucket_kernel<FB, true>), dim3((b.max_items * FB::LANES + 63) / 64, rows), dim3(64), 0, st, dev,
-                           b.offsets, b.counts, b.items, b.item_count, b.entries, b.partial_items, b.target, b.max_items, (const unsigned long long *)b.entry_base);
-    else
-        hipLaunchKernelGGL((frw::nmsm_bucket_kernel<FB, false>), dim3((b.max_items * FB::LANES + 63) / 64, rows), dim3(64), 0, st, dev,
-                           b.offsets, b.counts, b.items, b.item_count, b.entries, b.partial_items, b.target, b.max_items, (const unsigned long long *)b.entry_base);
-    hipLaunchKernelGGL(frw::nmsm_combine_kernel<FB>, dim3(frw::NMSM_BUCKETS, rows), dim3(64), 0, st, b.counts, b.offsets, b.item_first,
-                       b.partial_items, b.bucket_sums, b.target, b.max_items, (uint32_t)frw::NMSM_W);
-    hipLaunchKernelGGL(frw::nmsm_finish_kernel<FB>, dim3(rows), dim3(64), 0, st, b.counts, b.offsets, b.item_first, b.partial_items,
-                       b.bucket_sums, ones_for_finish, (int)ones_groups, ones_finish_stride, b.target, b.max_items,
-                       b.window_sums, 1, (uint32_t)frw::NMSM_W, 1);
-    hipLaunchKernelGGL(frw::msm_horner_kernel<FB>, dim3((unsigned)tables), dim3(64), 0, st, b.window_sums, frw::NMSM_W, frw::NMSM_C, d_out, xyzz_out ? 1 : 0,
-                       out_step);
+    const dim3 g_bucket((b.max_items * FB::LANES + 63) / 64, rows);
+    f = fl.take(g_bucket);
+    if constexpr (TWO)
+        hipLaunchKernelGGL((frw::nmsm_bucket_kernel<FB, false, false>), g_bucket, dim3(64), 0, st, dev, b.offsets, b.counts, b.items, b.item_count, b.entries,
+                           b.partial_items, b.target, b.max_items, (const unsigned long long *)b.entry_base, f);
+    hipLaunchKernelGGL((frw::nmsm_bucket_kernel<FB, PREFETCH && !TWO, true>), g_bucket, dim3(64), 0, st, dev, b.offsets, b.counts, b.items, b.item_count, b.entries,
+                       b.partial_items, b.target, b.max_items, (const unsigned long long *)b.entry_base, f);
+    const dim3 g_comb(frw::NMSM_BUCKETS, rows);
+    f = fl.take(g_comb);
+    if constexpr (TWO)
+        hipLaunchKernelGGL((frw::nmsm_combine_kernel<FB, false>), g_comb, dim3(64), 0, st, b.counts, b.offsets, b.item_first, b.partial_items, b.bucket_sums,
+                           b.target, b.max_items, (uint32_t)frw::NMSM_W, f);
+    hipLaunchKernelGGL((frw::nmsm_combine_kernel<FB, true>), g_comb, dim3(64), 0, st, b.counts, b.offsets, b.item_first, b.partial_items, b.bucket_sums,
+                       b.target, b.max_items, (uint32_t)frw::NMSM_W, f);
+    const dim3 g_fin(rows);
+    f = fl.take(g_fin);
+    if constexpr (TWO)
+        hipLaunchKernelGGL((frw::nmsm_finish_kernel<FB, false>), g_fin, dim3(64), 0, st, b.counts, b.offsets, b.item_first, b.partial_items, b.bucket_sums,
+                           ones_for_finish, (int)ones_groups, ones_finish_stride, b.target, b.max_items, b.window_sums, 1, (uint32_t)frw::NMSM_W, 1, f);
+    hipLaunchKernelGGL((frw::nmsm_finish_kernel<FB, true>), g_fin, dim3(64), 0, st, b.counts, b.offsets, b.item_first, b.partial_items, b.bucket_sums,
+                       ones_for_finish, (int)ones_groups, ones_finish_stride, b.target, b.max_items, b.window_sums, 1, (uint32_t)frw::NMSM_W, 1, f);
+    const dim3 g_horner((unsigned)tables);
+    f = fl.take(g_horner);
+    if constexpr (TWO)
+        hipLaunchKernelGGL((frw::msm_horner_kernel<FB, false>), g_horner, dim3(64), 0, st, b.window_sums, frw::NMSM_W, frw::NMSM_C, d_out, xyzz_out ? 1 : 0, out_step, f);
+    hipLaunchKernelGGL((frw::msm_horner_kernel<FB, true>), g_horner, dim3(64), 0, st, b.window_sums, frw::NMSM_W, frw::NMSM_C, d_out, xyzz_out ? 1 : 0, out_step, f);
     return hipGetLastError();
 }
 template <class F, bool PREFETCH>
```

Measured after the change: 1.332 million, median of 6. About the same (-0.1%).
